# bowman-lab/enspara

Measured on AMD Instinct MI355X. Metric: frame x center RMSD pairs/sec in k-centers assign, higher is better.
Workload: dtype f32

## Files before the change

enspara_amd/_lib.py:

```python
import collections
import ctypes as C
import os

import numpy as np

HERE = os.path.dirname(os.path.abspath(__file__))
LIB_PATH = os.environ.get("ENSPARA_HIP_LIB",
                          os.path.join(HERE, "libenspara_hip.so"))

EK_TILE = 256
EK_OK, EK_EARG, EK_EHIP, EK_ESTATE, EK_ENOMEM = 0, -1, -2, -3, -4

SYMBOLS = [
    "ek_abi_version", "ek_last_error", "ek_device_count",
    "ek_ctx_create", "ek_ctx_destroy", "ek_ctx_sync", "ek_ctx_stream",
    "ek_load_frames", "ek_rmsd_to_center",
    "ek_state_reset", "ek_state_download", "ek_state_upload",
    "ek_record_bytes", "ek_local_candidate", "ek_own_record",
    "ek_kcenters_step", "ek_kcenters_run",
    "ek_history_download", "ek_history_reset",
    "ek_spec_candidates", "ek_round_candidates", "ek_quad_copy_ready",
    "ek_spec_begin", "ek_spec_round", "ek_spec_localmax",
    "ek_spec_apply", "ek_spec_round_end", "ek_spec_progress", "ek_spec_rounds",
    "ek_spec_chain_bytes", "ek_spec_chain_rows", "ek_spec_chain_max",
    "ek_spec_chain_apply", "ek_run_stats", "ek_ti_stats", "ek_view_stats",
    "ek_last_run_form",
    "ek_view_layout_check",
    "ek_ms_setup", "ek_ms_mailbox", "ek_ms_connect", "ek_ms_begin", "ek_ms_local",
    "ek_ms_global", "ek_ms_end", "ek_ms_run", "ek_ms_state", "ek_ms_diag",
    "ek_assign_nearest",
    "ek_pam_begin", "ek_pam_count_members", "ek_pam_select_member",
    "ek_pam_propose", "ek_pam_propose_member", "ek_pam_commit",
    "ek_pam_count_members_batch", "ek_pam_select_members_batch",
    "ek_pam_prefetch", "ek_pam_propose_ex", "ek_pam_prefetch_stats",
    "ek_pam_prefetch_window", "ek_pam_prefetch_passes", "ek_pam_sparse_stats", "ek_pam_ahead_stats", "ek_pam_window_run", "ek_pam_sweep", "ek_np_choice_draws",
    "ek_pam_window_max",
    "ek_pam_prefetch_centers_window",
    "ek_centered_frames", "ek_pam_begin_table", "ek_pam_prefetch_centers",
    "ek_pam_propose_center",
    "ek_msm_counts", "ek_msm_counts_ctx", "ek_msm_row_normalize",
    "ek_msm_mle_prinz", "ek_msm_bace_prune", "ek_msm_bace_run",
    "ek_msm_boot_open", "ek_msm_boot_fetch", "ek_msm_boot_build", "ek_msm_boot_last_timing",
    "ek_msm_boot_close",
    "ek_lu_solve", "ek_lu_set_timing", "ek_lu_last_timing",
    "ek_tpt_committors", "ek_tpt_mfpts_sinks", "ek_tpt_mfpts_all", "ek_tpt_fluxes",
    "ek_mi_open", "ek_mi_add", "ek_mi_load_counts", "ek_mi_counts", "ek_mi_information",
    "ek_mi_last_timing", "ek_mi_close",
    "ek_cards_open", "ek_cards_add", "ek_cards_stats", "ek_cards_disorder",
    "ek_cards_disorder_codes", "ek_cards_matrices", "ek_cards_counts",
    "ek_cards_last_timing", "ek_cards_close", "ek_cards_scan_chunk",
    "ek_sasa_open", "ek_sasa_run", "ek_sasa_last_timing", "ek_sasa_close",
    "ek_rmsf_open", "ek_rmsf_run", "ek_rmsf_fetch", "ek_rmsf_last_timing", "ek_rmsf_close",
    "ek_wmi_run", "ek_wmi_last_timing",
    "ek_ent_kl_rows", "ek_ent_js_rows", "ek_ent_shannon_rows", "ek_ent_kl_counts",
    "ek_ent_last_timing", "ek_ent_state_counts_open", "ek_ent_state_counts_add",
    "ek_ent_state_counts_read", "ek_ent_state_counts_last_timing",
    "ek_ent_state_counts_close",
    "ek_kmc_create", "ek_kmc_destroy", "ek_kmc_next", "ek_kmc_trajectories",
    "ek_kmc_ensemble", "ek_kmc_fret_probs", "ek_kmc_fret_bursts", "ek_kmc_last_timing",
    "ek_dye_pair_create", "ek_dye_pair_destroy", "ek_dye_pair_table", "ek_dye_pair_resolve",
    "ek_dye_pair_static", "ek_dye_pair_last_timing",
    "ek_dye_bursts_lifetimes", "ek_dye_bursts_k2", "ek_dye_photons_lifetimes",
    "ek_dye_photons_k2", "ek_dye_pick_events", "ek_dye_bursts_last_timing",
    "ek_pockets_open", "ek_pockets_run", "ek_pockets_counts", "ek_pockets_fetch",
    "ek_pockets_last_timing", "ek_pockets_close", "ek_pockets_touches", "ek_pockets_ranks",
    "ek_pockets_labels",
    "ek_dyes_open", "ek_dyes_run", "ek_dyes_counts", "ek_dyes_fetch", "ek_dyes_last_timing",
    "ek_dyes_close", "ek_dyes_touches", "ek_dyes_pair_hist",
    "ek_rotamer_states", "ek_dihedral_angles", "ek_dihedral_rotamers",
    "ek_krylov_create", "ek_krylov_destroy", "ek_krylov_set_vector",
    "ek_krylov_get_vector", "ek_krylov_step", "ek_krylov_rotate",
    "ek_krylov_combine", "ek_krylov_expand", "ek_krylov_set_filter",
    "ek_feat_create", "ek_feat_destroy", "ek_feat_load", "ek_feat_distance",
    "ek_feat_kcenters", "ek_feat_pam_sweep", "ek_feat_pam_release",
    "ek_feat_record_bytes", "ek_feat_create_sharded", "ek_feat_state_reset",
    "ek_feat_state_upload", "ek_feat_state_download", "ek_feat_local_candidate",
    "ek_feat_kcenters_step", "ek_feat_history_download", "ek_feat_history_reset",
    "ek_feat_pam_count_batch", "ek_feat_pam_select_batch", "ek_feat_pam_gather_rows",
    "ek_feat_pam_begin", "ek_feat_pam_propose", "ek_feat_pam_commit",
    "ek_feat_assign_nearest",
    "ek_set_frames_per_lane", "ek_set_option", "ek_get_option", "ek_last_run_timing",
    "ek_reserve_centers",
    "ek_debug_guards",
    "ek_timing_begin", "ek_timing_end", "ek_timing_form", "ek_hbm_copy_rate",
    "ek_qcp_probe", "ek_pam_pairs_probe",
    "ek_live_resources", "ek_fail_alloc_at",
]


EK_OPT_NONTEMPORAL = 1
EK_OPT_ASSIGN_KERNEL = 2
EK_OPT_CANDIDATES = 4
EK_OPT_CHAINED = 5
EK_OPT_PAM_PRUNE = 6
EK_OPT_STATE_EXACT = 7
EK_OPT_ADAPTIVE = 8
EK_OPT_PASS_FORM = 9
EK_OPT_FUSED_ROUNDS = 10
EK_OPT_TRIANGLE = 11
EK_OPT_PAM_ONE_WORKGROUP = 12
EK_OPT_PAM_MAX_PAIRS = 13
EK_OPT_PAM_BOTH_SUMS = 14
EK_OPT_FINE_PICK = 15
EK_OPT_PAM_BOUNDS = 16
EK_OPT_PICK_CAP = 17
EK_OPT_SMALL_SHARDS = 18
EK_OPT_PAM_AHEAD = 19
EK_OPT_PAM_ZERO_COPY = 20
EK_OPT_PAM_PAIRS_MFMA = 21
EK_OPT_PASS_SWEEP = 22
EK_OPT_MS_TWO_PHASE = 23
EK_OPT_ACTIVE_VIEW = 24
EK_OPT_VIEW_RHO = 25
EK_OPT_VIEW_RATIO = 26
OPTIONS = {k[7:].lower(): v for k, v in list(globals().items())
           if k.startswith("EK_OPT_")}


class HipLibraryMissing(RuntimeError):
    pass


class HipError(RuntimeError):
    pass


_lib = None


def load():
    global _lib
    if _lib is not None:
        return _lib
    if not os.path.exists(LIB_PATH):
        raise HipLibraryMissing(
            "%s not found: the HIP extension is not built "
            "(run `python -m enspara_amd.build`); there is no CPU fallback."
            % LIB_PATH)
    if os.environ.get("ENSPARA_NO_TORCH") != "1":
        try:
            import torch
        except Exception:
            pass
    try:
        L = C.CDLL(LIB_PATH, mode=C.RTLD_GLOBAL)
    except OSError as e:
        raise HipLibraryMissing("cannot load %s: %s" % (LIB_PATH, e))
    vp, i32, i64, f32 = C.c_void_p, C.c_int32, C.c_int64, C.c_float
    f32p, i32p, i64p = (C.POINTER(C.c_float), C.POINTER(C.c_int32),
                        C.POINTER(C.c_int64))
    L.ek_abi_version.restype = C.c_int
    L.ek_last_error.restype = C.c_char_p
    L.ek_device_count.restype = C.c_int
    L.ek_ctx_create.argtypes = [C.c_int, i64, i32, i64, vp, C.POINTER(vp)]
    L.ek_ctx_destroy.argtypes = [vp]
    L.ek_ctx_sync.argtypes = [vp]
    L.ek_ctx_stream.restype = vp
    L.ek_ctx_stream.argtypes = [vp]
    L.ek_load_frames.argtypes = [vp, vp, i64, i64, C.c_int]
    L.ek_rmsd_to_center.argtypes = [vp, i64, f32p, f32p]
    L.ek_state_reset.argtypes = [vp]
    L.ek_state_download.argtypes = [vp, f32p, i32p]
    L.ek_state_upload.argtypes = [vp, f32p, i32p]
    L.ek_record_bytes.restype = C.c_size_t
    L.ek_record_bytes.argtypes = [i32]
    L.ek_local_candidate.argtypes = [vp, vp]
    L.ek_own_record.restype = vp
    L.ek_own_record.argtypes = [vp]
    L.ek_kcenters_step.argtypes = [vp, vp, i32, i32, C.c_double, vp]
    L.ek_kcenters_run.argtypes = [vp, i32, i32, C.c_double, i32p, i64p, f32p, f32p]
    L.ek_history_download.argtypes = [vp, i32, i32, i64p, f32p, i32p]
    L.ek_history_reset.argtypes = [vp]
    L.ek_spec_candidates.argtypes = [vp]
    L.ek_round_candidates.argtypes = [vp]
    L.ek_quad_copy_ready.argtypes = [vp]
    L.ek_spec_begin.argtypes = [vp, i32, i32, vp]
    L.ek_spec_round.argtypes = [vp, vp, i32, C.c_double]
    L.ek_spec_localmax.argtypes = [vp, vp]
    L.ek_spec_apply.argtypes = [vp, vp, i32, C.c_double]
    L.ek_spec_chain_bytes.argtypes = [i32p, i32p]
    L.ek_spec_chain_rows.argtypes = [vp, vp]
    L.ek_spec_chain_max.argtypes = [vp, vp, i32, vp]
    L.ek_spec_chain_apply.argtypes = [vp, vp, i32, C.c_double]
    L.ek_spec_round_end.argtypes = [vp, vp]
    L.ek_spec_progress.argtypes = [vp, i32p, i32p]
    L.ek_spec_rounds.argtypes = [vp, i32p]
    L.ek_run_stats.argtypes = [vp, i64p, i64p]
    L.ek_ms_setup.argtypes = [vp, i32, i32, C.POINTER(C.c_size_t)]
    L.ek_ms_mailbox.argtypes = [vp, C.POINTER(vp), C.POINTER(vp), vp, vp]
    L.ek_ms_connect.argtypes = [vp, i32, vp, vp, vp, vp]
    L.ek_ms_begin.argtypes = [vp, i32, i32]
    L.ek_ms_local.argtypes = [vp, C.c_double, vp]
    L.ek_ms_global.argtypes = [vp, C.c_double, vp]
    L.ek_ms_end.argtypes = [vp]
    L.ek_ms_state.argtypes = [vp, i32p, i32p, i32p]
    L.ek_ms_run.argtypes = [vp, i32, i32, C.c_double, i32p, i64p, f32p, f32p]
    L.ek_ti_stats.argtypes = [vp, i64p, i64p]
    L.ek_view_stats.argtypes = [vp, i64p]
    L.ek_last_run_form.argtypes = [vp, i64p]
    L.ek_view_layout_check.argtypes = [vp, f32, i64p]
    L.ek_assign_nearest.argtypes = [vp, f32p, i32]
    f64p = C.POINTER(C.c_double)
    L.ek_ms_diag.argtypes = [vp, i64p, f64p]
    L.ek_pam_begin.argtypes = [vp, i64p, i32]
    L.ek_pam_count_members.argtypes = [vp, i32, i64p]
    L.ek_pam_select_member.argtypes = [vp, i32, i64, i64p]
    L.ek_pam_propose.argtypes = [vp, i32, i64, f64p, f64p, i64p]
    L.ek_pam_propose_member.argtypes = [vp, i32, i64, i64p, f64p, f64p, i64p]
    L.ek_pam_commit.argtypes = [vp, C.c_int]
    L.ek_pam_count_members_batch.argtypes = [vp, i32, i32, i64p]
    L.ek_pam_select_members_batch.argtypes = [vp, i32, i32, i64p, i64p]
    L.ek_pam_prefetch.argtypes = [vp, i64p, i32]
    L.ek_pam_propose_ex.argtypes = [vp, i32, i64, i64, i32, i32, f64p, f64p,
                                    i64p, C.POINTER(C.c_uint32)]
    L.ek_pam_prefetch_stats.argtypes = [vp, i64p, i64p]
    L.ek_pam_window_run.argtypes = [vp, i32, i32, i64p, i64p, i32, i32, i32p, i32p,
                                    f64p, f64p, i64p]
    L.ek_pam_window_max.argtypes = []
    L.ek_pam_window_max.restype = i32
    L.ek_pam_prefetch_window.argtypes = [vp, i64p, i32, i32, i32]
    L.ek_pam_prefetch_passes.argtypes = [vp, i64p, i64p]
    L.ek_pam_sparse_stats.argtypes = [vp, i64p, i64p]
    L.ek_pam_ahead_stats.argtypes = [vp, i64p]
    L.ek_np_choice_draws.argtypes = [C.POINTER(C.c_uint32), i64, i64p, i64p, i64, i64p]
    L.ek_np_choice_draws.restype = i64
    L.ek_pam_sweep.argtypes = [vp, i32, i32, C.POINTER(C.c_uint32), i64, i64p, i64p, i32p, i64p,
                               i32p, f64p, f64p, i64p, i32p]
    L.ek_pam_prefetch_centers_window.argtypes = [vp, vp, vp, i32, i32, i32]
    L.ek_centered_frames.argtypes = [vp, i64p, i32p, i32, vp, vp]
    L.ek_pam_begin_table.argtypes = [vp, vp, vp, i32]
    L.ek_pam_prefetch_centers.argtypes = [vp, vp, vp, i32]
    L.ek_pam_propose_center.argtypes = [vp, i32, i32, vp, vp, i64, i32, i32, vp]
    L.ek_msm_counts.argtypes = [C.c_int, i32p, i64p, i64, i32, i32, i32, i64,
                                i32p, i32p, i64p, i64p]
    L.ek_msm_counts_ctx.argtypes = [vp, i64p, i64, i32, i32, i32, i64, i32p, i32p,
                                    i64p, i64p]
    L.ek_msm_row_normalize.argtypes = [C.c_int, i64p, f64p, i64, f64p, f64p]
    L.ek_msm_mle_prinz.argtypes = [C.c_int, i32, i64, i32, i64p, i32p, i32p, f64p,
                                   f64p, f64p, f64p, f64p, f64p, f64p, C.c_double,
                                   i64, i64p, f64p]
    L.ek_msm_bace_prune.argtypes = [C.c_int, i32, f64p, f64p, f32p]
    L.ek_msm_bace_run.argtypes = [C.c_int, i32, f64p, f64p, i32p, i32, i32, i32, vp,
                                  i32, f32p]
    L.ek_msm_boot_open.argtypes = [C.c_int, i32p, i64p, i64, i32, i32, i32, i64, i64p, i32p,
                                   i32, i32p, i32, C.POINTER(vp)]
    L.ek_msm_boot_fetch.argtypes = [vp, i32, i32, i64p]
    L.ek_msm_boot_build.argtypes = [vp, i64, i64p, i64p, i64p, f64p, f64p]
    L.ek_msm_boot_last_timing.argtypes = [vp, f64p]
    L.ek_msm_boot_close.argtypes = [vp]
    L.ek_lu_solve.argtypes = [C.c_int, i32, f64p, i32, f64p, f64p, i32p, i32p]
    L.ek_lu_set_timing.argtypes = [C.c_int]
    L.ek_lu_last_timing.argtypes = [f64p, f64p]
    L.ek_tpt_committors.argtypes = [C.c_int, i32, f64p, i32p, i32, i32p, i32, f64p, i32p]
    L.ek_tpt_mfpts_sinks.argtypes = [C.c_int, i32, f64p, i32p, i32, C.c_double, f64p, i32p]
    L.ek_tpt_mfpts_all.argtypes = [C.c_int, i32, f64p, f64p, C.c_double, f64p, i32p]
    L.ek_tpt_fluxes.argtypes = [C.c_int, i32, f64p, i32p, i32, i32p, i32, f64p, i32, f64p,
                                f64p, i32p]
    u8p, u32p = C.POINTER(C.c_uint8), C.POINTER(C.c_uint32)
    L.ek_mi_open.argtypes = [C.c_int, i32, i32, i32, i32, C.POINTER(vp)]
    L.ek_mi_add.argtypes = [vp, u8p, u8p, i64]
    L.ek_mi_load_counts.argtypes = [vp, u32p, C.c_uint64]
    L.ek_mi_counts.argtypes = [vp, u32p]
    L.ek_mi_information.argtypes = [vp, f64p]
    L.ek_mi_last_timing.argtypes = [vp, f64p]
    L.ek_mi_close.argtypes = [vp]
    L.ek_cards_open.argtypes = [C.c_int, i32, i32, C.POINTER(vp)]
    L.ek_cards_add.argtypes = [vp, u8p, i64]
    L.ek_cards_stats.argtypes = [vp, i64p]
    L.ek_cards_disorder.argtypes = [vp, i64p, i64p]
    L.ek_cards_disorder_codes.argtypes = [vp, i32, u8p]
    L.ek_cards_matrices.argtypes = [vp, f64p]
    L.ek_cards_counts.argtypes = [vp, i32, u32p]
    L.ek_cards_last_timing.argtypes = [vp, f64p]
    L.ek_cards_close.argtypes = [vp]
    L.ek_cards_scan_chunk.argtypes = []
    L.ek_cards_scan_chunk.restype = C.c_int
    L.ek_sasa_open.argtypes = [C.c_int, i32, f32p, i32, f32p, i32, i32p, i32p, C.POINTER(vp)]
    L.ek_sasa_run.argtypes = [vp, f32p, i64, i64, i32p, f32p, f32p]
    L.ek_sasa_last_timing.argtypes = [vp, f64p]
    L.ek_sasa_close.argtypes = [vp]
    L.ek_rmsf_open.argtypes = [C.c_int, i32, i32, i32p, f32p, i32, i32p, i32p, C.POINTER(vp)]
    L.ek_rmsf_run.argtypes = [vp, f32p, i64, f64p, i64, i64, f32p, f64p, f32p,
                              C.POINTER(C.c_uint32)]
    L.ek_rmsf_fetch.argtypes = [vp, f64p, f64p]
    L.ek_rmsf_last_timing.argtypes = [vp, f64p]
    L.ek_rmsf_close.argtypes = [vp]
    L.ek_wmi_run.argtypes = [C.c_int, u8p, f64p, i64, i32, i32, f64p, f64p]
    L.ek_wmi_last_timing.argtypes = [f64p]
    L.ek_ent_kl_rows.argtypes = [C.c_int, i64, i64, f64p, f64p, f64p, u32p]
    L.ek_ent_js_rows.argtypes = [C.c_int, i64, i64, f64p, f64p, f64p, f64p, u32p]
    L.ek_ent_shannon_rows.argtypes = [C.c_int, i64, i64, f64p, i32, f64p]
    L.ek_ent_kl_counts.argtypes = [C.c_int, i32, f64p, i64, i32p, i32p, i64p, C.c_double,
                                   f64p, u32p]
    L.ek_ent_last_timing.argtypes = [f64p]
    L.ek_ent_state_counts_open.argtypes = [C.c_int, i32, i32, C.POINTER(vp)]
    L.ek_ent_state_counts_add.argtypes = [vp, u8p, i64]
    L.ek_ent_state_counts_read.argtypes = [vp, C.POINTER(C.c_uint64)]
    L.ek_ent_state_counts_last_timing.argtypes = [vp, f64p]
    L.ek_ent_state_counts_close.argtypes = [vp]
    u64 = C.c_uint64
    L.ek_kmc_create.argtypes = [C.c_int, i32, i64p, i32p, f64p, C.POINTER(vp)]
    L.ek_kmc_destroy.argtypes = [vp]
    L.ek_kmc_next.argtypes = [vp, i64, i32p, f64p, i32p, i64p]
    L.ek_kmc_trajectories.argtypes = [vp, u64, i64, i64, i32p, i64, i32, i64, i32p, i64p]
    L.ek_kmc_ensemble.argtypes = [C.c_int, i32, f64p, i64p, i32p, f64p, f64p, i64, f64p,
                                  f64p, f64p]
    L.ek_kmc_fret_probs.argtypes = [C.c_int, u64, i64, i64, i32p, i32, i64p, f64p, f64p,
                                    C.c_double, C.c_double, f64p]
    L.ek_kmc_fret_bursts.argtypes = [vp, u64, i64, i64, i64p, i64p, f64p, i64p, f64p, f64p,
                                     C.c_double, C.c_double, i64, u8p, i32p, i64p]
    L.ek_kmc_last_timing.argtypes = [f64p]
    i8p = C.POINTER(C.c_int8)
    L.ek_dye_pair_create.argtypes = [C.c_int, i32, i64p, i64p, i32p, f64p, f64p, f64p, i64p,
                                     i64p, i32p, f64p, f64p, f64p, f64p, C.POINTER(vp)]
    L.ek_dye_pair_destroy.argtypes = [vp]
    L.ek_dye_pair_table.argtypes = [vp, i32, f64p, f64p, f64p, f64p]
    L.ek_dye_pair_resolve.argtypes = [vp, u64, i64, i64, i64, i64, i32p, i8p, i32p, i32p, i64,
                                      i64p, i64p]
    L.ek_dye_pair_static.argtypes = [vp, u64, i64, i64, f64p, i8p, i32p, i32p]
    L.ek_dye_pair_last_timing.argtypes = [f64p]
    L.ek_dye_bursts_lifetimes.argtypes = [vp, u64, i64, i64, i64p, i64p, f64p, i64p, f64p, u8p,
                                          i64, u8p, f64p, i32p, i32p, i64p, i64p]
    L.ek_dye_bursts_k2.argtypes = [vp, u64, i64, i64, i64p, i64p, f64p, i64p, f64p, i64p, f64p,
                                   C.c_double, i64, u8p, f64p, f64p, i32p, i32p, i32p, i32p,
                                   i64p, i64p]
    L.ek_dye_photons_lifetimes.argtypes = [C.c_int, u64, i64, i64, i32p, i32, i64p, f64p, u8p,
                                           u8p, f64p, i64p]
    L.ek_dye_photons_k2.argtypes = [C.c_int, u64, i64, i64, i32p, i32, i64p, f64p, i64p, f64p,
                                    C.c_double, u8p, f64p, f64p, i32p, i32p, i64p]
    L.ek_dye_pick_events.argtypes = [C.c_int, i64, i32p, f64p, i32, i64p, i64p, i64p]
    L.ek_dye_bursts_last_timing.argtypes = [f64p]
    L.ek_pockets_open.argtypes = [C.c_int, i32, f64p, C.c_double, i32, C.POINTER(vp)]
    L.ek_pockets_run.argtypes = [vp, f32p, i64, f32p, i32p, i64]
    L.ek_pockets_counts.argtypes = [vp, i64, i64p]
    L.ek_pockets_fetch.argtypes = [vp, i32p, i32p]
    L.ek_pockets_last_timing.argtypes = [vp, f64p]
    L.ek_pockets_close.argtypes = [vp]
    L.ek_pockets_touches.argtypes = [C.c_int, f32p, i32, f64p, C.c_double, f32p, i32p, u8p]
    L.ek_pockets_ranks.argtypes = [C.c_int, u8p, i32p, u8p]
    L.ek_pockets_labels.argtypes = [C.c_int, u8p, i32p, i32p]
    L.ek_dyes_open.argtypes = [C.c_int, i32, f64p, i32, f32p, i32, f32p, C.c_double,
                               C.POINTER(vp)]
    L.ek_dyes_run.argtypes = [vp, f32p, i64, f32p, i64]
    L.ek_dyes_counts.argtypes = [vp, i64, i32p, i32p]
    L.ek_dyes_fetch.argtypes = [vp, i64p]
    L.ek_dyes_last_timing.argtypes = [vp, f64p]
    L.ek_dyes_close.argtypes = [vp]
    L.ek_dyes_touches.argtypes = [C.c_int, f32p, i32, f64p, f32p, i32, u8p]
    L.ek_dyes_pair_hist.argtypes = [C.c_int, f32p, i32, f32p, i32, C.c_double, i32p, i64p]
    L.ek_rotamer_states.argtypes = [C.c_int, f32p, i64, i32, u8p, i32, i32p, f64p, f32p,
                                    C.c_double, u8p, f64p]
    L.ek_dihedral_angles.argtypes = [C.c_int, f32p, i64, i32, i32p, i32, f32p, f64p]
# ... 113 lines not shown
```

enspara_amd/csrc/ek_api.hip:

```cpp
#include "ek_ctx.h"
#include "ek_view.h"
#include <cmath>
#include <mutex>
#include "ek_qcp.h"

static thread_local char g_err[512] = "";

int ek_set_error(int code, const char *fmt, ...)
{
    va_list ap;
    va_start(ap, fmt);
    vsnprintf(g_err, sizeof(g_err), fmt, ap);
    va_end(ap);
    return code;
}
void ek_ctx_msm_view(ek_ctx *c, int *device, int64_t *n, const int32_t **assign,
                     hipStream_t *stream, void ***scratch_slot)
{
    *device = c->device;
    *n = c->loaded ? c->n : -1;
    *assign = c->assign;
    *stream = c->stream;
    *scratch_slot = &c->msm_scratch;
}
// ... 125 lines not shown
    for (size_t k = 0; k < g_uc_live.size(); ++k)
        if (g_uc_live[k].ptr == ptr && g_uc_live[k].device == device) {
            g_uc_free.push_back(g_uc_live[k]);
            g_uc_live.erase(g_uc_live.begin() + k);
            return;
        }
}

bool ek_poison()
{
    static const bool on = getenv("EK_POISON") != nullptr;
    return on;
}
hipError_t ek_malloc_named(ek_ctx *c, void **ptr, size_t bytes, const char *name)
{
    if (!ek_poison())
        return ek_dev_malloc(ptr, bytes);
    hipError_t e = ek_dev_malloc(ptr, bytes + EK_GUARD_BYTES);
    static const int fill = getenv("EK_POISON_BYTE") ? (int)strtol(getenv("EK_POISON_BYTE"), nullptr, 0)
                                                     : 0x5a;
    if (e == hipSuccess)
        e = hipMemset(*ptr, fill, bytes);
    if (e == hipSuccess)
        e = hipMemset((unsigned char *)*ptr + bytes, 0xA5, EK_GUARD_BYTES);
    if (e == hipSuccess)
        e = hipDeviceSynchronize();
    if (e == hipSuccess)
        c->guards.push_back({name, (unsigned char *)*ptr + bytes});
    return e;
}
extern "C" int ek_debug_guards(ek_ctx *c)
{
    if (!c)
        return ek_fail(EK_EARG, "NULL context");
    EK_HIP(hipSetDevice(c->device));
    EK_HIP(hipDeviceSynchronize());
    int bad = 0;
    std::vector<unsigned char> h(EK_GUARD_BYTES);
    for (const ek_ctx::Guard &g : c->guards) {
        if (hipMemcpy(h.data(), g.at, EK_GUARD_BYTES, hipMemcpyDeviceToHost) != hipSuccess) {
            (void)hipGetLastError();
            continue;
        }
        for (size_t k = 0; k < h.size(); ++k)
            if (h[k] != 0xA5) {
                fprintf(stderr, "enspara_hip: buffer %s overrun: byte + %zu behind its end "
                                "is 0x%02x\n", g.name, k, h[k]);
                ++bad;
                break;
            }
    }
    return bad;
}

int ek_spec_alloc(ek_ctx *c)
{
    if (!c->top)
        EK_HIP(ek_malloc_named(c, (void **)&c->top, ek_top_scratch_bytes(c->A), "top"));
    if (!c->planD)
        EK_HIP(ek_malloc_named(c, (void **)&c->planD, 64 * 64 * sizeof(float), "planD"));
    if (!c->pm) {
        const size_t nb = ((size_t)std::max<int64_t>(c->n, 1) + EK_BLOCK - 1) /
                          EK_BLOCK;
        if (!c->fm)
            EK_HIP(ek_malloc_named(c, (void **)&c->fm, 4 * nb * sizeof(EkBlockMax), "fm"));
        EK_HIP(ek_malloc_named(c, (void **)&c->pm,
                               (size_t)(EK_MAX_CANDS - 1) * nb * sizeof(EkBlockMax), "pm"));
    }
    if (!c->vecs) {
        const size_t bytes = (size_t)(EK_MAX_CANDS - 1) * std::max<int64_t>(c->n_pad, 1) *
                             sizeof(float);
        EK_HIP(ek_malloc_named(c, (void **)&c->vecs, bytes, "vecs"));
    }
    return EK_OK;
}

extern "C" int ek_abi_version(void) { return EK_ABI_VERSION; }
extern "C" const char *ek_last_error(void) { return g_err; }

extern "C" int ek_device_count(void)
{
    int n = 0;
    hipError_t e = hipGetDeviceCount(&n);
    if (e != hipSuccess)
        return ek_fail(EK_EHIP, "hipGetDeviceCount: %s", hipGetErrorString(e));
    return n;
}

extern "C" size_t ek_record_bytes(int32_t n_atoms) { return ek_rec_bytes(n_atoms); }

int ek_free_all(ek_ctx *c)
{
    if (!c)
        return EK_OK;
    (void)hipSetDevice(c->device);
    if (c->stream)
        (void)hipStreamSynchronize(c->stream);
    (void)ek_dev_free(c->tiles);
    (void)ek_dev_free(c->qtiles);
    (void)ek_dev_free(c->aos);
    (void)ek_dev_free(c->G);
    (void)ek_dev_free(c->dist);
    (void)ek_dev_free(c->assign);
    (void)ek_dev_free(c->scratch);
    (void)ek_dev_free(c->rec);
    (void)ek_dev_free(c->rec_tmp);
    (void)ek_dev_free(c->blockmax);
    (void)ek_dev_free(c->hist);
    (void)ek_dev_free(c->ctl);
    for (int b = 0; b < 2; ++b) {
        (void)ek_dev_free(c->stage[b]);
        (void)ek_pinned_free(c->pin[b]);
        if (c->up_ev[b])
            (void)ek_event_destroy(c->up_ev[b]);
    }
    delete c->pool;
    (void)ek_dev_free(c->cen_aos);
    (void)ek_dev_free(c->cen_G);
    (void)ek_dev_free(c->cen_tiles);
    (void)ek_dev_free(c->cen_blocks);
    (void)ek_dev_free(c->bat_blockcnt);
    (void)ek_dev_free(c->bat_scan);
    (void)ek_dev_free(c->bat_sel);
    (void)ek_dev_free(c->pam_vecs);
    (void)ek_dev_free(c->pam_recs);
    (void)ek_dev_free(c->pam_plan);
    (void)ek_dev_free(c->moved);
    (void)ek_dev_free(c->tmp_idx);
    (void)ek_dev_free(c->pam_out_dev);
    (void)ek_dev_free(c->med_list);
    (void)ek_dev_free(c->dtab);
    if (c->act_n_host)
        (void)ek_pinned_free(c->act_n_host);
    if (c->pam_out_host)
        (void)ek_pinned_free(c->pam_out_host);
    (void)ek_dev_free(c->pam_win_dev);
    (void)ek_dev_free(c->sp_buf);
    (void)ek_dev_free(c->act_list);
    if (c->pam_win_host)
        (void)ek_pinned_free(c->pam_win_host);
    ek_msm_scratch_free(c->msm_scratch);
    for (void *m : c->ms_ipc)
        (void)hipIpcCloseMemHandle(m);
    (void)ek_dev_free(c->ms);
    ek_uncached_free(c->device, c->ms_mbox);
    ek_uncached_free(c->device, c->ms_flags);
    (void)ek_dev_free(c->recsT);
    (void)ek_dev_free(c->ctile);
    (void)ek_dev_free(c->ctrace);
    (void)ek_dev_free(c->ti_D);
    (void)ek_dev_free(c->ti_tab);
    (void)ek_dev_free(c->ti_tabG);
    (void)ek_dev_free(c->ti_skip);
    (void)ek_dev_free(c->ti_stats);
    (void)ek_dev_free(c->pend);
    (void)ek_dev_free(c->ord);
    (void)ek_dev_free(c->tick);
    (void)ek_dev_free(c->rows);
    (void)ek_dev_free(c->vmask);
    (void)ek_dev_free(c->plan);
    (void)ek_dev_free(c->vecs);
    (void)ek_dev_free(c->hdr);
    (void)ek_dev_free(c->pm);
    (void)ek_dev_free(c->ti_rtab);
    (void)ek_dev_free(c->ti_tmask);
    (void)ek_dev_free(c->pam_dprop);
    (void)ek_pinned_free(c->sel_host);
    (void)ek_pinned_free(c->cnt_host);
    (void)ek_pinned_free(c->js_host);
    (void)ek_dev_free(c->sp_marks);
    if (c->win_ev)
        (void)ek_event_destroy(c->win_ev);
    (void)ek_dev_free(c->fm);
    ek_view_free(c);
    (void)ek_dev_free(c->top);
    (void)ek_dev_free(c->planD);
    (void)ek_dev_free(c->ndist);
    (void)ek_dev_free(c->nassign);
    (void)ek_dev_free(c->amb);
    (void)ek_dev_free(c->amb_best);
    (void)ek_dev_free(c->amb_count);
    (void)ek_dev_free(c->blockcnt);
    (void)ek_dev_free(c->scan);
    (void)ek_dev_free(c->sel);
    (void)ek_dev_free(c->sq_part);
    (void)ek_dev_free(c->pw_shapes);
    (void)ek_dev_free(c->sq_out);
    (void)ek_dev_free(c->med_aos);
    (void)ek_dev_free(c->med_G);
    (void)ek_dev_free(c->med_idx);
    (void)ek_dev_free(c->ambt);
    (void)ek_dev_free(c->ambG);
    for (hipEvent_t e : c->samp_ev)
        (void)ek_event_destroy(e);
    if (c->ev0)
        (void)ek_event_destroy(c->ev0);
    if (c->ev1)
        (void)ek_event_destroy(c->ev1);
    if (c->evb0)
        (void)ek_event_destroy(c->evb0);
    if (c->evb1)
        (void)ek_event_destroy(c->evb1);
    if (c->own_stream && c->stream)
        (void)ek_stream_destroy(c->stream);
    delete c;
    return EK_OK;
}

extern "C" int ek_ctx_create(int device, int64_t n_frames, int32_t n_atoms,
                             int64_t global_offset, void *stream, ek_ctx **out)
{
    if (!out)
        return ek_fail(EK_EARG, "ek_ctx_create: out is NULL");
    *out = nullptr;
    if (n_frames < 0 || n_frames > 0x7fffff00LL)
        return ek_fail(EK_EARG, "ek_ctx_create: n_frames=%lld out of range",
                       (long long)n_frames);
    if (n_atoms < 1 || n_atoms > EK_MAX_ATOMS)
        return ek_fail(EK_EARG, "ek_ctx_create: n_atoms=%d out of range [1,%d]",
                       n_atoms, EK_MAX_ATOMS);
    EK_HIP(hipSetDevice(device));
    ek_ctx *c = new (std::nothrow) ek_ctx();
    if (!c)
        return ek_fail(EK_ENOMEM, "ek_ctx_create: out of host memory");
    c->device = device;
    c->n = n_frames;
    c->A = n_atoms;
    c->goff = global_offset;
    c->n_tiles = (n_frames + EK_TILE - 1) / EK_TILE;
    if (stream) {
        c->stream = (hipStream_t)stream;
    } else {
        hipError_t e = ek_stream_create_flags(&c->stream, hipStreamNonBlocking);
        if (e != hipSuccess) {
            delete c;
            return ek_fail(EK_EHIP, "ek_ctx_create: creating the stream: %s", hipGetErrorString(e));
        }
        c->own_stream = true;
    }
    const size_t tile_floats = (size_t)3 * n_atoms * EK_TILE;
    const size_t nn = (size_t)std::max<int64_t>(n_frames, 1);
    const size_t nt = (size_t)std::max<int64_t>(c->n_tiles, 1);
    const size_t recb = ek_rec_bytes(n_atoms);
    c->blockmax_cap = (int)((n_frames + EK_BLOCK - 1) / EK_BLOCK) + 1;
    c->hist_cap = 1024;
    hipError_t e = hipSuccess;
#define EK_ALLOC(ptr, bytes)                                                   \
    if (e == hipSuccess)                                                       \
        e = ek_malloc_named(c, (void **)&(ptr), (bytes), #ptr);
    EK_ALLOC(c->tiles, nt * tile_floats * sizeof(float));
    EK_ALLOC(c->aos, nn * (size_t)3 * n_atoms * sizeof(float));
    EK_ALLOC(c->G, nn * sizeof(double));
    EK_ALLOC(c->dist, nn * sizeof(float));
    EK_ALLOC(c->assign, nn * sizeof(int32_t));
    EK_ALLOC(c->scratch, nn * sizeof(float));
    EK_ALLOC(c->rec, recb);
    EK_ALLOC(c->rec_tmp, recb);
    EK_ALLOC(c->blockmax, (size_t)c->blockmax_cap * sizeof(EkBlockMax));
    EK_ALLOC(c->hist, (size_t)c->hist_cap * sizeof(EkHist));
    EK_ALLOC(c->ctl, sizeof(EkCtl));
    EK_ALLOC(c->recsT, recb * EK_MAX_CANDS);
    EK_ALLOC(c->plan, sizeof(EkPlan));
    EK_ALLOC(c->hdr, sizeof(EkMaxHdr));
    EK_ALLOC(c->pend, sizeof(EkPend));
    EK_ALLOC(c->ord, sizeof(EkChainOrd));
#ifdef EK_P16_STATS
    EK_ALLOC(c->tick, (256 + 64 * 16 + 2048) * sizeof(unsigned int));
    (void)hipMemset(c->tick, 0, (256 + 64 * 16 + 2048) * sizeof(unsigned int));
#else
    EK_ALLOC(c->tick, 256 * sizeof(unsigned int));
#endif
    EK_ALLOC(c->rows, EK_MAX_CANDS * sizeof(EkChainRow));
    EK_ALLOC(c->vmask, (nt * EK_TILE / EK_WAVE) * sizeof(uint32_t));
    EK_ALLOC(c->ctile, ek_ctile_bytes(n_atoms));
    EK_ALLOC(c->ctrace, EK_MAX_CANDS * sizeof(double));
#undef EK_ALLOC
    c->n_pad = (int64_t)nt * EK_TILE;
    if (e == hipSuccess)
        e = ek_event_create(&c->ev0);
    if (e == hipSuccess)
        e = ek_event_create(&c->ev1);
    if (e == hipSuccess && c->n_tiles > 0)
        e = hipMemsetAsync(c->tiles + (size_t)(c->n_tiles - 1) * tile_floats, 0,
                           tile_floats * sizeof(float), c->stream);
    if (e == hipSuccess)
        e = hipMemsetAsync(c->hist, 0, (size_t)c->hist_cap * sizeof(EkHist),
                           c->stream);
    if (e == hipSuccess)
        e = hipMemsetAsync(c->ctl, 0, sizeof(EkCtl), c->stream);
    if (e == hipSuccess)
        e = hipMemsetAsync(c->rec, 0, recb, c->stream);
    if (e == hipSuccess)
        e = hipMemsetAsync(c->pend, 0, sizeof(EkPend), c->stream);
    if (e == hipSuccess)
        e = hipMemsetAsync(c->plan, 0, sizeof(EkPlan), c->stream);
    if (e == hipSuccess)
        e = hipMemsetAsync(c->ord, 0, sizeof(EkChainOrd), c->stream);
    if (e == hipSuccess)
        e = hipMemsetAsync(c->tick, 0, 256 * sizeof(unsigned int), c->stream);
    if (e == hipSuccess)
        e = hipMemsetAsync(c->rows, 0, EK_MAX_CANDS * sizeof(EkChainRow),
                           c->stream);
    if (e != hipSuccess) {
        ek_free_all(c);
        return ek_fail(e == hipErrorOutOfMemory ? EK_ENOMEM : EK_EHIP,
                       "ek_ctx_create: %s", hipGetErrorString(e));
    }
    *out = c;
    return EK_OK;
}

extern "C" int ek_ctx_destroy(ek_ctx *ctx) { return ek_free_all(ctx); }

extern "C" int ek_ctx_sync(ek_ctx *c)
{
    if (!c)
        return ek_fail(EK_EARG, "NULL context");
    EK_HIP(hipSetDevice(c->device));
    EK_HIP(hipStreamSynchronize(c->stream));
    return EK_OK;
}

extern "C" void *ek_ctx_stream(ek_ctx *c) { return c ? (void *)c->stream : nullptr; }
extern "C" void *ek_own_record(ek_ctx *c) { return c ? (void *)c->rec : nullptr; }

extern "C" int ek_set_frames_per_lane(ek_ctx *c, int fpl)
{
    if (!c)
        return ek_fail(EK_EARG, "NULL context");
    if (fpl != 0 && fpl != 1 && fpl != 2 && fpl != 4)
        return ek_fail(EK_EARG, "frames per lane must be 0, 1, 2 or 4");
    c->fpl = fpl;
    return EK_OK;
}

extern "C" int ek_set_option(ek_ctx *c, int32_t key, int32_t value)
{
    if (!c)
        return ek_fail(EK_EARG, "NULL context");
    switch (key) {
    case EK_OPT_NONTEMPORAL:
        c->nt = value < 0 ? -1 : (value ? 1 : 0);
        return EK_OK;
    case EK_OPT_CANDIDATES:
        if (value != -1 && value != 1 && value != 4 && value != 8 && value != 16 &&
            value != 32)
            return ek_fail(EK_EARG, "ek_set_option: candidates per round must "
                                    "be -1 (auto), 1, 4, 8, 16 or 32");
        c->cands = value;
        return EK_OK;
    case EK_OPT_CHAINED:
        if (value != 0 && value != 1)
            return ek_fail(EK_EARG, "ek_set_option: chained rounds 0 or 1");
        c->chain = value;
        return EK_OK;
    case EK_OPT_PAM_PRUNE:
        if (value != 0 && value != 1)
            return ek_fail(EK_EARG, "ek_set_option: PAM medoid pruning 0 or 1");
        c->prune = value;
        return EK_OK;
    case EK_OPT_STATE_EXACT:
        if (value != 0 && value != 1)
            return ek_fail(EK_EARG, "ek_set_option: state-is-exact flag 0 or 1");
        c->state_exact = value != 0;
        return EK_OK;
    case EK_OPT_TRIANGLE:
        if (value != 0 && value != 1)
            return ek_fail(EK_EARG, "ek_set_option: triangle inequality 0 or 1");
        c->tri = value;
        return EK_OK;
    case EK_OPT_FUSED_ROUNDS:
        if (value != 0 && value != 1)
            return ek_fail(EK_EARG, "ek_set_option: fused rounds 0 or 1");
        c->fused = value;
        return EK_OK;
    case 9:
        if (value != 1)
            return ek_fail(EK_EARG, "ek_set_option: pass kernel form must be 1");
        return EK_OK;
    case EK_OPT_ADAPTIVE:
        if (value != 0 && value != 1)
            return ek_fail(EK_EARG, "ek_set_option: adaptive candidates 0 or 1");
        c->adapt = value;
        return EK_OK;
    case EK_OPT_PAM_ONE_WORKGROUP:
        if (value != 0 && value != 1)
            return ek_fail(EK_EARG, "ek_set_option: one-workgroup PAM windows 0 or 1");
        c->pam_sparse = value;
        return EK_OK;
    case EK_OPT_PAM_BOTH_SUMS:
        if (value != 0 && value != 1)
            return ek_fail(EK_EARG, "ek_set_option: both cost sums for every proposal 0 or 1");
        c->sp_exact = value;
        return EK_OK;
    case EK_OPT_PAM_MAX_PAIRS:
        if (value < 0)
            return ek_fail(EK_EARG, "ek_set_option: pairs one workgroup searches >= 0");
        c->sp_max_pairs = value;
        return EK_OK;
    case EK_OPT_PAM_PAIRS_MFMA:
        if (value != 0 && value != 1)
            return ek_fail(EK_EARG, "ek_set_option: PAM pairs kernels on the matrix cores 0 or 1");
        ek_pam_pairs_form = value;
        return EK_OK;
    case EK_OPT_PAM_ZERO_COPY:
        if (value != 0 && value != 1)
            return ek_fail(EK_EARG, "ek_set_option: PAM results into mapped host memory 0 or 1");
        c->pam_zero_copy = value;
        return EK_OK;
    case EK_OPT_PAM_AHEAD:
        if (value != 0 && value != 1)
            return ek_fail(EK_EARG, "ek_set_option: PAM slots evaluated ahead 0 or 1");
        c->pam_spec = value;
        return EK_OK;
    case EK_OPT_SMALL_SHARDS:
        if (value != 0 && value != 1)
            return ek_fail(EK_EARG, "ek_set_option: small shards 0 or 1");
        c->ms_small = value;
        return EK_OK;
    case EK_OPT_PICK_CAP:
        if (value < 0 || value > 16)
            return ek_fail(EK_EARG, "ek_set_option: far frames per label on the pick's list "
                                    "0 (by the yield) or 1 .. 16");
        c->pick_cap = value;
        return EK_OK;
    case EK_OPT_PAM_BOUNDS:
        if (value != 0 && value != 1)
            return ek_fail(EK_EARG, "ek_set_option: PAM tables as bounds 0 or 1");
        c->pam_bounds = value;
        return EK_OK;
    case EK_OPT_FINE_PICK:
        if (value != 0 && value != 1)
            return ek_fail(EK_EARG, "ek_set_option: maxima per 64 frames for the pick 0 or 1");
        c->fine_pick = value;
        return EK_OK;
    case EK_OPT_MS_TWO_PHASE:
        if (value != 0 && value != 1)
            return ek_fail(EK_EARG, "ek_set_option: headers first in the mailbox rounds 0 or 1");
        c->ms_two_phase = value;
        return EK_OK;
    case EK_OPT_PASS_SWEEP:
        if (value < 0 || value > 2)
// ... 247 lines not shown
        return ek_fail(EK_EARG, "NULL context");
    if (!c->loaded)
        return ek_fail(EK_ESTATE, "ek_state_reset: no frames loaded");
    EK_HIP(hipSetDevice(c->device));
    ek_launch_fill_state(c->dist, c->assign, c->n, __builtin_inff(), -1,
                         c->stream);
    EK_CHECK_LAUNCH();
    c->state_exact = true;
    ek_pam_forget(c);
    int rc = ek_history_reset(c);
    if (rc)
        return rc;
    return ek_local_candidate(c, nullptr);
}

extern "C" int ek_state_download(ek_ctx *c, float *dist_host,
                                 int32_t *assign_host)
{
    if (!c)
        return ek_fail(EK_EARG, "NULL context");
    EK_HIP(hipSetDevice(c->device));
    if (dist_host && c->n)
        EK_HIP(hipMemcpyAsync(dist_host, c->dist, (size_t)c->n * sizeof(float),
                              hipMemcpyDeviceToHost, c->stream));
    if (assign_host && c->n)
        EK_HIP(hipMemcpyAsync(assign_host, c->assign,
                              (size_t)c->n * sizeof(int32_t),
                              hipMemcpyDeviceToHost, c->stream));
    EK_HIP(hipStreamSynchronize(c->stream));
    return EK_OK;
}

extern "C" int ek_state_upload(ek_ctx *c, const float *dist_host,
                               const int32_t *assign_host)
{
    if (!c || !dist_host || !assign_host)
        return ek_fail(EK_EARG, "ek_state_upload: NULL argument");
    EK_HIP(hipSetDevice(c->device));
    if (c->n) {
        EK_HIP(hipMemcpyAsync(c->dist, dist_host, (size_t)c->n * sizeof(float),
                              hipMemcpyHostToDevice, c->stream));
        EK_HIP(hipMemcpyAsync(c->assign, assign_host,
                              (size_t)c->n * sizeof(int32_t),
                              hipMemcpyHostToDevice, c->stream));
    }
    EK_HIP(hipStreamSynchronize(c->stream));
    c->state_exact = false;
    ek_pam_forget(c);
    return ek_local_candidate(c, nullptr);
}

extern "C" int ek_local_candidate(ek_ctx *c, void *rec_dev)
{
    if (!c)
        return ek_fail(EK_EARG, "NULL context");
    if (!c->loaded)
        return ek_fail(EK_ESTATE, "ek_local_candidate: no frames loaded");
    EK_HIP(hipSetDevice(c->device));
    unsigned char *rec = rec_dev ? (unsigned char *)rec_dev : c->rec;
    ek_launch_pick(nullptr, 0, c->dist, c->tiles, c->G, c->n, c->A, c->goff,
                   rec, c->ctl, c->stream);
    EK_CHECK_LAUNCH();
    return EK_OK;
}

int ek_ensure_hist(ek_ctx *c, int32_t label)
{
    if (label < c->hist_cap)
        return EK_OK;
    int32_t cap = c->hist_cap;
    while (cap <= label)
        cap *= 2;
    EkHist *h = nullptr;
    hipError_t e = ek_dev_malloc((void **)&h, (size_t)cap * sizeof(EkHist));
    if (e == hipSuccess)
        e = hipMemsetAsync(h, 0, (size_t)cap * sizeof(EkHist), c->stream);
    if (e == hipSuccess)
        e = hipMemcpyAsync(h, c->hist, (size_t)c->hist_cap * sizeof(EkHist),
                           hipMemcpyDeviceToDevice, c->stream);
    if (e == hipSuccess)
        e = hipStreamSynchronize(c->stream);
    if (e != hipSuccess) {
        (void)hipStreamSynchronize(c->stream);
        (void)ek_dev_free(h);
        EK_HIP(e);
    }
    (void)ek_dev_free(c->hist);
    c->hist = h;
    c->hist_cap = cap;
    return EK_OK;
}

extern "C" int ek_kcenters_step(ek_ctx *c, const void *recs_dev, int32_t n_recs,
                                int32_t label, double dist_cutoff,
                                void *own_rec_out)
{
    if (!c)
        return ek_fail(EK_EARG, "NULL context");
    if (!c->loaded)
        return ek_fail(EK_ESTATE, "ek_kcenters_step: no frames loaded");
    if (label < 0)
        return ek_fail(EK_EARG, "ek_kcenters_step: negative label");
    EK_HIP(hipSetDevice(c->device));
    int rc = ek_ensure_hist(c, label);
    if (rc)
        return rc;
    const unsigned char *recs =
        recs_dev ? (const unsigned char *)recs_dev : c->rec;
    if (!recs_dev)
        n_recs = 1;
    if (n_recs < 1)
        return ek_fail(EK_EARG, "ek_kcenters_step: n_recs < 1");
    unsigned char *own = own_rec_out ? (unsigned char *)own_rec_out : c->rec;
    const int fpl = ek_pick_fpl(c);
    bool tri = false;
    if (c->tri && recs_dev && c->state_exact && c->A >= 3) {
        if (label == 0)
            c->ti_tab_n = 0;
        if (c->ti_tab_n == label) {
            if (label + 1 > c->ti_tab_cap) {
                const int32_t cap = std::max(2 * c->ti_tab_cap, std::max(label + 1, 256));
                float *t2 = nullptr, *d2 = nullptr;
                double *g2 = nullptr;
                EK_HIP(ek_wait(c));
                hipError_t e = ek_dev_malloc((void **)&t2, (size_t)cap * 3 * c->A * sizeof(float));
                if (e == hipSuccess)
                    e = ek_dev_malloc((void **)&g2, (size_t)cap * sizeof(double));
                if (e == hipSuccess)
                    e = ek_dev_malloc((void **)&d2, (size_t)cap * sizeof(float));
                if (e == hipSuccess && c->ti_tab_n > 0)
                    e = hipMemcpy(t2, c->ti_tab, (size_t)c->ti_tab_n * 3 * c->A * sizeof(float),
                                  hipMemcpyDeviceToDevice);
                if (e == hipSuccess && c->ti_tab_n > 0)
                    e = hipMemcpy(g2, c->ti_tabG, (size_t)c->ti_tab_n * sizeof(double),
                                  hipMemcpyDeviceToDevice);
                if (e != hipSuccess) {
                    (void)ek_dev_free(t2);
                    (void)ek_dev_free(g2);
                    (void)ek_dev_free(d2);
                    EK_HIP(e);
                }
                (void)ek_dev_free(c->ti_tab);
                (void)ek_dev_free(c->ti_tabG);
                (void)ek_dev_free(c->ti_D);
                c->ti_tab = t2;
                c->ti_tabG = g2;
                c->ti_D = d2;
                c->ti_tab_cap = cap;
                c->ti_cap = cap;
            }
            if (!c->ti_skip)
                EK_HIP(ek_dev_malloc((void **)&c->ti_skip,
                                     (size_t)std::max<int64_t>(c->n_tiles, 1)));
            if (!c->ti_stats) {
                EK_HIP(ek_dev_malloc((void **)&c->ti_stats, 2 * sizeof(unsigned long long)));
                EK_HIP(hipMemsetAsync(c->ti_stats, 0, 2 * sizeof(unsigned long long),
                                      c->stream));
            }
            if (label == 0)
                EK_HIP(hipMemsetAsync(c->ti_stats, 0, 2 * sizeof(unsigned long long),
                                      c->stream));
            ek_launch_ti_tab(c->ti_tab, c->ti_tabG, c->A, label, recs, n_recs, c->ti_D,
                             c->dist, c->assign, c->n, c->ctl, c->ti_skip, c->ti_stats,
                             c->stream);
            EK_CHECK_LAUNCH();
            c->ti_tab_n = label + 1;
            tri = label >= 1 && c->n > 0;
        }
    }
    if (c->n > 0) {
        const bool sample =
            c->samp_every > 0 && (c->samp_count++ % c->samp_every) == 0 &&
            2 * (size_t)c->samp_used + 1 < c->samp_ev.size();
        if (sample)
        c->samp_form[c->samp_used] = 1;
    if (sample)
            EK_HIP(hipEventRecord(c->samp_ev[2 * c->samp_used], c->stream));
        ek_launch_step(fpl, 0, ek_pick_nt(c), c->tiles, c->G, c->dist, c->assign, c->scratch,
                       recs, n_recs, c->n, c->A, label, dist_cutoff,
                       c->blockmax, c->hist, c->ctl, c->stream,
                       tri ? c->ti_skip : nullptr);
        EK_CHECK_LAUNCH();
        if (sample) {
            EK_HIP(hipEventRecord(c->samp_ev[2 * c->samp_used + 1], c->stream));
            c->samp_used++;
        }
    }
    ek_launch_pick(c->n > 0 ? c->blockmax : nullptr,
                   ek_step_blocks(fpl, c->n), c->dist, c->tiles, c->G, c->n,
                   c->A, c->goff, own, c->ctl, c->stream);
    EK_CHECK_LAUNCH();
    return EK_OK;
}

extern "C" int ek_history_download(ek_ctx *c, int32_t first, int32_t count,
                                   int64_t *center_index_out,
                                   float *center_dist_out, int32_t *n_done)
{
    if (!c)
        return ek_fail(EK_EARG, "NULL context");
    if (first < 0 || count < 0)
        return ek_fail(EK_EARG, "ek_history_download: bad range");
    EK_HIP(hipSetDevice(c->device));
    EkCtl ctl;
    EK_HIP(hipMemcpyAsync(&ctl, c->ctl, sizeof(ctl), hipMemcpyDeviceToHost,
                          c->stream));
    std::vector<EkHist> h;
    const int32_t avail = std::max(0, std::min(count, c->hist_cap - first));
    if (avail > 0) {
        h.resize(avail);
        EK_HIP(hipMemcpyAsync(h.data(), c->hist + first,
                              (size_t)avail * sizeof(EkHist),
                              hipMemcpyDeviceToHost, c->stream));
    }
    EK_HIP(ek_wait(c));
    for (int32_t i = 0; i < count; ++i) {
        const bool ok = i < avail && h[i].set;
        if (center_index_out)
            center_index_out[i] = ok ? h[i].gidx : -1;
        if (center_dist_out)
            center_dist_out[i] = ok ? h[i].dist : 0.f;
    }
    if (n_done)
        *n_done = ctl.n_done;
    return EK_OK;
}

extern "C" int ek_timing_begin(ek_ctx *c, int32_t sample_every,
                               int32_t max_samples)
{
    if (!c || sample_every < 1 || max_samples < 1)
        return ek_fail(EK_EARG, "ek_timing_begin: bad argument");
    EK_HIP(hipSetDevice(c->device));
    while (c->samp_ev.size() < 2 * (size_t)max_samples) {
        hipEvent_t e;
        EK_HIP(ek_event_create(&e));
        c->samp_ev.push_back(e);
    }
    c->samp_form.assign((size_t)max_samples, 0);
    c->samp_every = sample_every;
    c->samp_used = 0;
    c->samp_count = 0;
    return EK_OK;
}

extern "C" int ek_timing_end(ek_ctx *c, float *avg_ms, int32_t *n_samples)
{
    if (!c)
        return ek_fail(EK_EARG, "NULL context");
    EK_HIP(hipSetDevice(c->device));
    EK_HIP(ek_wait(c));
    int cnt[EK_MAX_CANDS + 1] = {0};
    for (int i = 0; i < c->samp_used; ++i)
        cnt[std::min(std::max(c->samp_form[i], 0), EK_MAX_CANDS)]++;
    int dom = 0;
    for (int f = 1; f <= EK_MAX_CANDS; ++f)
        if (cnt[f] > cnt[dom])
            dom = f;
    c->samp_dom = dom;
    std::vector<float> t((size_t)c->samp_used);
    float mx = 0.f;
    for (int i = 0; i < c->samp_used; ++i) {
        EK_HIP(hipEventElapsedTime(&t[i], c->samp_ev[2 * i],
                                   c->samp_ev[2 * i + 1]));
        if (c->samp_form[i] == dom)
            mx = std::max(mx, t[i]);
    }
    double sum = 0.0;
    int used = 0;
    for (int i = 0; i < c->samp_used; ++i)
        if (c->samp_form[i] == dom && t[i] > 0.25f * mx) {
            sum += t[i];
            ++used;
        }
    if (avg_ms)
        *avg_ms = used ? (float)(sum / used) : 0.f;
    if (n_samples)
        *n_samples = used;
    c->samp_every = 0;
    return EK_OK;
}

extern "C" int ek_timing_form(ek_ctx *c, int32_t *candidates)
{
    if (!c || !candidates)
        return ek_fail(EK_EARG, "ek_timing_form: NULL argument");
    *candidates = c->samp_dom;
    return EK_OK;
}

extern "C" int ek_assign_nearest(ek_ctx *c, const float *centers_xyz,
                                 int32_t n_centers)
{
    if (!c || (!centers_xyz && n_centers > 0))
        return ek_fail(EK_EARG, "ek_assign_nearest: NULL argument");
    if (!c->loaded)
        return ek_fail(EK_ESTATE, "ek_assign_nearest: no frames loaded");
    if (n_centers < 0)
        return ek_fail(EK_EARG, "ek_assign_nearest: negative n_centers");
    if ((size_t)3 * c->A * 8 * sizeof(float) > 150 * 1024)
        return ek_fail(EK_EARG, "ek_assign_nearest: %d atoms exceed the LDS "
                                "center tile (limit 1600)", c->A);
    EK_HIP(hipSetDevice(c->device));
    c->state_exact = false;
    ek_pam_forget(c);
    if (n_centers > 0) {
        int rc = ek_upload_centers(c, centers_xyz, n_centers);
        if (rc)
            return rc;
    }
    const bool mfma = c->assign_variant == 2 || c->assign_variant == 3 ||
// ... 211 lines not shown
```

enspara_amd/csrc/ek_api_run.hip:

```cpp
#include "ek_ctx.h"
#include "ek_run_policy.h"
#include "ek_view.h"
#include <cmath>

void ek_view_free(ek_ctx *c)
{
    (void)ek_dev_free(c->v_aos);
    (void)ek_dev_free(c->v_tiles);
    (void)ek_dev_free(c->v_qtiles);
    (void)ek_dev_free(c->v_G);
    (void)ek_dev_free(c->v_dist);
    (void)ek_dev_free(c->v_assign);
    (void)ek_dev_free(c->v_act);
    (void)ek_dev_free(c->v_blockcnt);
    (void)ek_dev_free(c->v_blockoff);
    (void)ek_dev_free(c->v_count);
    c->v_aos = c->v_tiles = c->v_qtiles = nullptr;
    c->v_G = nullptr;
    c->v_dist = nullptr;
    c->v_assign = nullptr;
    c->v_act = c->v_blockcnt = c->v_blockoff = c->v_count = nullptr;
    c->view_cap = 0;
}

// ... 3 lines not shown
    if (c->view_cap >= cap)
        return EK_OK;
    EK_HIP(ek_wait(c));
    ek_view_free(c);
    const size_t nt = (size_t)(cap / EK_TILE), A3 = (size_t)3 * c->A;
    const size_t nblk = ek_view_sel_blocks(std::max<int64_t>(c->n, 1));
    hipError_t e = hipSuccess;
#define EK_VALLOC(ptr, bytes)                                                  \
    if (e == hipSuccess)                                                       \
        e = ek_malloc_named(c, (void **)&(ptr), (bytes), #ptr);
    EK_VALLOC(c->v_aos, (size_t)cap * A3 * sizeof(float));
    EK_VALLOC(c->v_tiles, nt * A3 * EK_TILE * sizeof(float));
    EK_VALLOC(c->v_qtiles, ek_quad_tiles_bytes((int64_t)nt, c->A));
    EK_VALLOC(c->v_G, (size_t)cap * sizeof(double));
    EK_VALLOC(c->v_dist, (size_t)cap * sizeof(float));
    EK_VALLOC(c->v_assign, (size_t)cap * sizeof(int32_t));
    EK_VALLOC(c->v_act, (size_t)cap * sizeof(uint32_t));
    EK_VALLOC(c->v_blockcnt, nblk * sizeof(uint32_t));
    EK_VALLOC(c->v_blockoff, nblk * sizeof(uint32_t));
    EK_VALLOC(c->v_count, 2 * sizeof(uint32_t));
    if (e == hipSuccess)
        e = hipMemsetAsync(c->v_count, 0, 2 * sizeof(uint32_t), c->stream);
#undef EK_VALLOC
    if (e != hipSuccess) {
        (void)hipGetLastError();
        ek_view_free(c);
        if (e == hipErrorOutOfMemory) {
            c->view_nomem = true;
            return EK_ENOMEM;
        }
        EK_HIP(e);
    }
    c->view_cap = cap;
    return EK_OK;
}

struct EkViewRun {
    bool on = false;
    int64_t n = 0;
    int32_t label_lo = 0;
    double guard = 0.0;
    bool tiles_valid = false;
};

static hipError_t ek_view_poison(ek_ctx *c)
{
    const size_t cap = (size_t)c->view_cap, nt = cap / EK_TILE, A3 = (size_t)3 * c->A;
    hipError_t e = hipMemsetAsync(c->v_aos, 0xFF, cap * A3 * sizeof(float), c->stream);
    if (e == hipSuccess)
        e = hipMemsetAsync(c->v_tiles, 0xFF, nt * A3 * EK_TILE * sizeof(float), c->stream);
    if (e == hipSuccess)
        e = hipMemsetAsync(c->v_qtiles, 0xFF, ek_quad_tiles_bytes((int64_t)nt, c->A),
                           c->stream);
    if (e == hipSuccess)
        e = hipMemsetAsync(c->v_G, 0xFF, cap * sizeof(double), c->stream);
    if (e == hipSuccess)
        e = hipMemsetAsync(c->v_dist, 0xFF, cap * sizeof(float), c->stream);
    if (e == hipSuccess)
        e = hipMemsetAsync(c->v_assign, 0xFF, cap * sizeof(int32_t), c->stream);
    return e;
}

static bool ek_view_build(ek_ctx *c, int64_t n_v)
{
    ek_launch_view_build(c->v_act, n_v, c->A, c->qt_valid, c->aos, c->G, c->dist, c->assign,
                         c->v_aos, c->qt_valid ? c->v_qtiles : c->v_tiles, c->v_G, c->v_dist,
                         c->v_assign, c->stream);
    return !c->qt_valid;
}

static void ek_view_scatter_back(ek_ctx *c, EkViewRun &v)
{
    ek_launch_view_scatter(c->v_act, v.n, c->v_dist, c->v_assign, c->dist, c->assign,
                           c->hist, v.label_lo, c->hist_cap, c->ctl, c->goff, c->stream);
    v.on = false;
}

void ek_round_of(ek_ctx *c, int T, double cutoff, EkRound &R)
{
    R.dist = c->dist;
    R.assign = c->assign;
    R.vecs = c->vecs;
    R.n = c->n;
    R.n_pad = c->n_pad;
    R.goff = c->goff;
    R.A = c->A;
    R.T = T;
    R.tiles = c->tiles;
    R.qtiles = c->qtiles;
    R.aos = c->aos;
    R.G = c->G;
    R.recs = c->recsT;
    R.plan = c->plan;
    R.pend = c->pend;
    R.ord = c->ord;
    R.blockmax = c->blockmax;
    R.pm = c->pm;
    R.fm = c->fine_pick ? c->fm : nullptr;
    R.sweep = (c->pass_sweep == 2 ||
               (c->pass_sweep == 1 && ek_sweep_pays(c->n))) ? 1 : 0;
    R.top = c->top;
    R.ctile = c->ctile;
    R.ctrace = c->ctrace;
    R.hist = c->hist;
    R.ctl = c->ctl;
    R.tick = c->tick;
    R.rows = c->rows;
    R.vmask = c->vmask;
    R.cutoff = cutoff;
    R.pick_cap = c->pick_cap > 0 ? c->pick_cap : 4;
}

static void ek_note_run_form(ek_ctx *c, int fpl, int nt, bool fused, int Tmax, int sweep,
                             bool fine_buf)
{
    const int nb = (int)((c->n + EK_BLOCK - 1) / EK_BLOCK);
    const bool fine = fused && Tmax > 1 && fine_buf && ek_fine_fits(nb);
    c->last_form[0] = fpl;
    c->last_form[1] = nt ? 1 : 0;
    c->last_form[2] = sweep ? 1 : 0;
    c->last_form[3] = fine ? 1 : 0;
    c->last_form[4] = nb;
    c->last_form[5] = Tmax > 1 ? (fine ? 4 * (int64_t)nb : nb) : ek_step_blocks(fpl, c->n);
}

#define EK_RC(call)                                                            \
    do {                                                                       \
        const int rc_ = (call);                                                \
        if (rc_)                                                               \
            return rc_;                                                        \
    } while (0)

struct EkRun {
    ek_ctx *c;
    EkViewRun &view;
    int32_t first_label, goal;
    double dist_cutoff;
    bool tri;
    bool fused;
    int fpl, nt;
    int view_mode;
    bool forced;
    double rho, shrink;
    EkRound R;
    int nb = 0;
    EkFormLadder lad;
    EkPickCap cap;
    EkTriPause ti;
    EkViewPolicy vp;
    int held = -1;
    bool pending = false;
    bool masks_fresh = false;
    bool looked = false;
    uint32_t look_cnt[2] = {0, 0};
    EkCtl cr;
    double per_round;
    int32_t rounds_before = 0;
    EkRun(ek_ctx *c_, EkViewRun &view_, bool adaptive, bool tri_, int Tmax)
        : c(c_), view(view_), tri(tri_), lad(adaptive, tri_, Tmax), cap(c_->pick_cap),
          per_round(ek_per_round_guess(lad.form))
    {
        memset(&cr, 0, sizeof(cr));
    }
};

static int ek_run_reserve_tri(ek_ctx *c, int32_t goal)
{
    if (goal > c->ti_cap) {
        EK_HIP(ek_wait(c));
        (void)ek_dev_free(c->ti_D);
        c->ti_D = nullptr;
        c->ti_cap = 0;
        EK_HIP(ek_dev_malloc((void **)&c->ti_D, (size_t)(goal + 1) * sizeof(float)));
        c->ti_cap = goal + 1;
    }
    if (!c->ti_skip)
        EK_HIP(ek_dev_malloc((void **)&c->ti_skip,
                             (size_t)std::max<int64_t>(c->n_tiles, 1)));
    if (!c->ti_stats)
        EK_HIP(ek_dev_malloc((void **)&c->ti_stats, 2 * sizeof(unsigned long long)));
    EK_HIP(hipMemsetAsync(c->ti_stats, 0, 2 * sizeof(unsigned long long),
                          c->stream));
    if (goal > c->ti_rtab_cap) {
        EK_HIP(ek_wait(c));
        (void)ek_dev_free(c->ti_rtab);
        c->ti_rtab = nullptr;
        c->ti_rtab_cap = 0;
        EK_HIP(ek_dev_malloc((void **)&c->ti_rtab,
                         (size_t)(goal + 1) * EK_MAX_CANDS * sizeof(float)));
        c->ti_rtab_cap = goal + 1;
    }
    if (!c->ti_tmask)
        EK_HIP(ek_dev_malloc((void **)&c->ti_tmask,
                         (size_t)std::max<int64_t>(c->n_tiles, 1) * sizeof(uint32_t)));
    return EK_OK;
}

static void ek_run_use_store(EkRun &run, bool the_view)
{
    ek_ctx *c = run.c;
    EkRound &R = run.R;
    if (the_view) {
        R.dist = c->v_dist;
        R.assign = c->v_assign;
        R.tiles = c->v_tiles;
        R.qtiles = c->v_qtiles;
        R.aos = c->v_aos;
        R.G = c->v_G;
        R.n = run.view.n;
        R.n_pad = (run.view.n + EK_TILE - 1) / EK_TILE * EK_TILE;
    } else {
        R.dist = c->dist;
        R.assign = c->assign;
        R.tiles = c->tiles;
        R.qtiles = c->qtiles;
        R.aos = c->aos;
        R.G = c->G;
        R.n = c->n;
        R.n_pad = c->n_pad;
    }
    run.nb = (int)((R.n + EK_BLOCK - 1) / EK_BLOCK);
    R.sweep = (run.fused && (c->pass_sweep == 2 ||
                             (c->pass_sweep == 1 && ek_sweep_pays(R.n)))) ? 1 : 0;
    R.cutoff = the_view ? std::max(run.dist_cutoff, run.view.guard) : run.dist_cutoff;
}

static void ek_run_leave_view(EkRun &run)
{
    if (run.pending) {
        ek_launch_round_flush(run.R, run.c->stream);
        run.pending = false;
    }
    ek_view_scatter_back(run.c, run.view);
    ek_run_use_store(run, false);
}

static int ek_run_enter_view(EkRun &run, int32_t left)
{
    ek_ctx *c = run.c;
    EkViewRun &view = run.view;
    run.looked = false;
    const EkViewPlan p =
        run.vp.decide(run.cr.last_max, run.rho, run.shrink, run.look_cnt,
                      view.on ? view.n : 0, c->n, left, run.per_round, run.forced);
    if (!p.build)
        return EK_OK;
    if (view.on) {
        ek_run_leave_view(run);
    } else if (run.pending) {
        ek_launch_round_flush(run.R, c->stream);
        run.pending = false;
    }
    uint32_t nv = 0;
    ek_launch_view_select(c->dist, c->n, p.theta, c->v_blockcnt, c->v_blockoff, c->v_act,
                          c->view_cap, c->v_count, c->stream);
    EK_CHECK_LAUNCH();
    EK_HIP(hipMemcpyAsync(&nv, c->v_count, sizeof(nv), hipMemcpyDeviceToHost, c->stream));
    EK_HIP(ek_wait(c));
    if (nv > 0 && (int64_t)nv < c->n && (int64_t)nv <= c->view_cap) {
        view.n = nv;
        view.label_lo = run.cr.n_done;
        view.guard = p.guard;
        if (run.view_mode == 3)
            EK_HIP(ek_view_poison(c));
        view.tiles_valid = ek_view_build(c, view.n);
        EK_CHECK_LAUNCH();
        view.on = true;
        ek_run_use_store(run, true);
        EK_HIP(hipMemsetAsync(c->vmask, 0, (size_t)(run.R.n_pad / EK_WAVE) * sizeof(uint32_t),
                              c->stream));
        c->view_stats[0]++;
    }
    run.held = -1;
    return EK_OK;
}

static void ek_run_pick_records(EkRun &run, int form, bool with_masks)
{
    ek_ctx *c = run.c;
    const EkRound &R = run.R;
    if (form == 1) {
        ek_launch_pick(c->blockmax, run.nb, R.dist, R.tiles, R.G, R.n, c->A, c->goff,
                       c->recsT, c->ctl, c->stream);
    } else if (run.fused) {
        ek_launch_round_chain(R, 1, c->stream);
        ek_launch_round_next(R, 1, c->stream);
        if (with_masks) {
            ek_launch_round_ti(R, run.goal, c->stream);
            run.masks_fresh = R.tmask != nullptr;
        }
    } else {
        ek_launch_pickT(c->blockmax, run.nb, R.tiles, R.G, R.assign, c->A, form, c->goff,
                        c->recsT, c->ctl, c->top, c->stream);
    }
}

static int ek_run_bootstrap(EkRun &run, int form)
{
    ek_ctx *c = run.c;
    if (run.pending) {
        ek_launch_round_flush(run.R, c->stream);
        run.pending = false;
    } else if (run.held <= 1) {
        ek_launch_blockmax(run.R.dist, run.R.n, c->blockmax, c->stream);
    }
    ek_run_pick_records(run, form, true);
    EK_CHECK_LAUNCH();
    if (form != 1)
        run.per_round = ek_per_round_guess(form);
    run.held = form;
    return EK_OK;
}

static int ek_run_enqueue_steps(EkRun &run, int32_t batch)
{
    ek_ctx *c = run.c;
    const EkRound &R = run.R;
    for (int32_t r = 0; r < batch; ++r) {
        const int label = run.cr.n_done + r;
        const bool skip = run.tri && label >= 1;
        if (skip)
            ek_launch_ti(R.aos, R.G, c->A, c->hist, label, c->goff, c->recsT, c->ti_D, R.dist,
                         R.assign, R.n, c->ctl, c->ti_skip, c->ti_stats, c->stream);
        ek_launch_step(run.fpl, 0, run.nt, R.tiles, R.G, R.dist, R.assign, c->scratch,
                       c->recsT, 1, R.n, c->A, label, R.cutoff, c->blockmax, c->hist, c->ctl,
                       c->stream, skip ? c->ti_skip : nullptr);
        ek_launch_pick(c->blockmax, ek_step_blocks(run.fpl, R.n), R.dist, R.tiles, R.G, R.n,
                       c->A, c->goff, c->recsT, c->ctl, c->stream);
        EK_CHECK_LAUNCH();
    }
    return EK_OK;
}

static bool ek_run_sample(EkRun &run, int form)
{
    ek_ctx *c = run.c;
    const bool sample =
        !run.view.on && c->samp_every > 0 && (c->samp_count++ % c->samp_every) == 0 &&
        2 * (size_t)c->samp_used + 1 < c->samp_ev.size();
    if (sample)
        c->samp_form[c->samp_used] = form;
    return sample;
}

static int ek_run_enqueue_fused(EkRun &run, int form, int32_t batch)
{
    ek_ctx *c = run.c;
    const EkRound &R = run.R;
    for (int32_t r = 0; r < batch; ++r) {
        const bool sample = ek_run_sample(run, form);
        if (sample)
            EK_HIP(hipEventRecord(c->samp_ev[2 * c->samp_used], c->stream));
        ek_launch_round_pass(R, c->stream);
        if (sample) {
            EK_HIP(hipEventRecord(c->samp_ev[2 * c->samp_used + 1], c->stream));
            c->samp_used++;
        }
        ek_launch_round_chain(R, 0, c->stream);
        ek_launch_round_next(R, 0, c->stream);
        ek_launch_round_ti(R, run.goal, c->stream);
        EK_CHECK_LAUNCH();
        run.pending = true;
    }
    return EK_OK;
}

static int ek_run_enqueue_unfused(EkRun &run, int form, int32_t batch)
{
    ek_ctx *c = run.c;
    const EkRound &R = run.R;
    const int nb = run.nb;
    for (int32_t r = 0; r < batch; ++r) {
        const bool sample = ek_run_sample(run, form);
        ek_launch_plan(c->recsT, form, c->A, form, R.cutoff, c->planD, c->plan, c->hist,
                       c->ctl, c->stream);
        if (sample)
            EK_HIP(hipEventRecord(c->samp_ev[2 * c->samp_used], c->stream));
        ek_launch_pass(form, R.tiles, R.qtiles, R.G, R.dist, R.assign, c->vecs, R.n, R.n_pad,
                       c->A, c->recsT, c->plan, c->blockmax, c->ctile, c->ctrace, c->stream);
        if (sample) {
            EK_HIP(hipEventRecord(c->samp_ev[2 * c->samp_used + 1], c->stream));
            c->samp_used++;
        }
        if (c->chain) {
            ek_launch_chain_max(R.dist, c->vecs, R.n, R.n_pad, c->plan, c->pm, 1, c->goff,
                                c->stream);
            ek_launch_chain_decide_local(c->blockmax, c->pm, nb, ek_chain_max_blocks(R.n),
                                         c->goff, R.cutoff, c->plan, c->hist, c->ctl,
                                         c->stream);
            ek_launch_chain_apply(c->vecs, R.n, R.n_pad, R.dist, R.assign, c->plan,
                                  c->blockmax, c->stream);
        } else {
            for (int j = 1; j < form; ++j) {
                ek_launch_localmax_check(c->blockmax, nb, c->goff, R.cutoff, c->plan, c->hist,
                                         c->ctl, c->stream);
                ek_launch_apply(c->vecs, R.G, R.n, R.n_pad, c->A, R.dist, R.assign, c->plan,
                                c->blockmax, c->stream);
            }
        }
        ek_launch_pickT(c->blockmax, nb, R.tiles, R.G, R.assign, c->A, form, c->goff, c->recsT,
                        c->ctl, c->top, c->stream);
        EK_CHECK_LAUNCH();
    }
    return EK_OK;
}

static int ek_run_enqueue_batch(EkRun &run, int form, int32_t batch)
{
    const EkRound &R = run.R;
    if (R.tmask && !run.masks_fresh) {
        ek_launch_round_ti(R, run.goal, run.c->stream);
        run.masks_fresh = true;
    }
    if (!R.tmask)
        run.masks_fresh = false;
    if (form == 1)
        return ek_run_enqueue_steps(run, batch);
    return run.fused ? ek_run_enqueue_fused(run, form, batch)
                     : ek_run_enqueue_unfused(run, form, batch);
}

static int ek_run_carry_look(EkRun &run)
{
    ek_ctx *c = run.c;
    if (!run.view_mode || run.vp.pause.tick())
        return EK_OK;
    const int64_t want_cap =
        run.forced ? c->n : (int64_t)std::ceil(run.shrink * (double)c->n);
    if (ek_view_alloc(c, want_cap) != EK_OK) {
        (void)hipGetLastError();
        run.view_mode = 0;
        return EK_OK;
    }
    EK_HIP(hipMemsetAsync(c->v_count, 0, sizeof(run.look_cnt), c->stream));
    ek_launch_view_look(run.R.dist, run.R.n, c->ctl, run.rho, EK_VIEW_REL, EK_VIEW_ABS,
                        c->v_count, c->stream);
    if (run.view.on)
        ek_launch_view_look(c->dist, c->n, c->ctl, run.rho, EK_VIEW_REL, EK_VIEW_ABS,
                            c->v_count + 1, c->stream);
    EK_CHECK_LAUNCH();
    EK_HIP(hipMemcpyAsync(run.look_cnt, c->v_count, sizeof(run.look_cnt),
                          hipMemcpyDeviceToHost, c->stream));
    run.looked = true;
    return EK_OK;
}

static int ek_run_read_back(EkRun &run, int form, int32_t &got, int32_t &ran)
{
    ek_ctx *c = run.c;
    const bool one = form == 1, masks = run.R.tmask != nullptr;
    const int32_t before = run.cr.n_done;
    EK_HIP(hipMemcpyAsync(&run.cr, c->ctl, sizeof(run.cr), hipMemcpyDeviceToHost, c->stream));
    unsigned long long ti_now[2] = {0, 0};
    if (masks)
        EK_HIP(hipMemcpyAsync(ti_now, c->ti_stats, sizeof(ti_now), hipMemcpyDeviceToHost,
                              c->stream));
    EK_HIP(ek_wait(c));
    if (masks)
        run.ti.look(ti_now);
    else if (!one)
        run.ti.skipped();
    got = run.cr.n_done - before;
    ran = one ? got : run.cr.n_rounds - run.rounds_before;
    run.rounds_before = run.cr.n_rounds;
    c->st_rounds[ek_form_slot(form)] += ran;
    c->st_centers[ek_form_slot(form)] += got;
    c->view_stats[1] += (int64_t)ran * run.R.n;
    c->view_stats[2] += (int64_t)ran * (c->n - run.R.n);
    return EK_OK;
}

static int ek_run_leave_on_stop(EkRun &run)
{
    ek_ctx *c = run.c;
    if ((double)run.cr.last_max > run.dist_cutoff)
        c->view_stats[3]++;
    ek_run_leave_view(run);
    const int32_t zero = 0;
    EK_HIP(hipMemcpyAsync(&c->ctl->stopped, &zero, sizeof(zero), hipMemcpyHostToDevice,
                          c->stream));
    EK_HIP(ek_wait(c));
    run.cr.stopped = 0;
    run.held = -1;
    run.looked = false;
    return EK_OK;
}

static int ek_run_finish(EkRun &run, int32_t max_new, int32_t *n_added,
                         int64_t *center_index_out, float *center_dist_out,
                         float *final_maxdist)
{
    ek_ctx *c = run.c;
    const int form = run.lad.form;
    if (run.pending) {
        ek_launch_round_flush(run.R, c->stream);
        run.pending = false;
        EK_CHECK_LAUNCH();
    }
    if (run.view.on || (run.held < 0 && run.cr.n_done > run.first_label)) {
        if (run.view.on)
            ek_run_leave_view(run);
        ek_launch_blockmax(run.R.dist, run.R.n, c->blockmax, c->stream);
        run.R.T = form;
        ek_run_pick_records(run, form, false);
        EK_CHECK_LAUNCH();
        run.held = form;
        EK_HIP(hipMemcpyAsync(&run.cr, c->ctl, sizeof(run.cr), hipMemcpyDeviceToHost,
                              c->stream));
        EK_HIP(ek_wait(c));
    }
    if (run.tri) {
        unsigned long long st[2] = {0, 0};
        EK_HIP(hipMemcpyAsync(st, c->ti_stats, sizeof(st), hipMemcpyDeviceToHost, c->stream));
        EK_HIP(ek_wait(c));
        c->ti_tiles = (int64_t)st[0];
        c->ti_skipped = (int64_t)st[1];
    }
    EK_HIP(hipEventRecord(c->ev1, c->stream));
    EK_HIP(ek_wait(c));
    EK_HIP(hipEventElapsedTime(&c->last_ms, c->ev0, c->ev1));
    if (run.held == 1) {
        ek_launch_blockmax(c->dist, c->n, c->blockmax, c->stream);
        EK_CHECK_LAUNCH();
    }
    if (run.held >= 0)
        EK_HIP(hipMemcpyAsync(c->rec, c->recsT, ek_rec_bytes(c->A), hipMemcpyDeviceToDevice,
                              c->stream));
    EK_HIP(ek_wait(c));
    const int32_t added_t =
        std::min(max_new, std::max(0, run.cr.n_done - run.first_label));
    const int64_t passes = c->st_rounds[0] + c->st_rounds[1] + c->st_rounds[2] +
                           c->st_rounds[3] + 2 * c->st_rounds[4];
    c->last_launches = (int32_t)passes;
    c->last_passes = (int32_t)passes;
    if (n_added)
        *n_added = added_t;
    if (final_maxdist)
        *final_maxdist = run.cr.last_max;
    if (added_t > 0 && (center_index_out || center_dist_out))
        EK_RC(ek_history_download(c, run.first_label, added_t, center_index_out,
                                  center_dist_out, nullptr));
    return EK_OK;
}

static int ek_run_rounds_in(ek_ctx *c, int Tmax, int32_t first_label,
                            int32_t max_new, double dist_cutoff, int32_t *n_added,
                            int64_t *center_index_out, float *center_dist_out,
                            float *final_maxdist, EkViewRun &view)
{
    EK_RC(ek_spec_alloc(c));
    if (!c->evb0) {
        EK_HIP(ek_event_create(&c->evb0));
        EK_HIP(ek_event_create(&c->evb1));
    }
    const int32_t goal = first_label + max_new;
    EkCtl ctlw;
    memset(&ctlw, 0, sizeof(ctlw));
    ctlw.n_done = first_label;
    ctlw.limit = goal;
    EK_HIP(hipMemcpyAsync(c->ctl, &ctlw, sizeof(ctlw), hipMemcpyHostToDevice,
                          c->stream));
    EK_HIP(ek_wait(c));
    for (int m = 0; m < EK_N_FORMS; ++m)
        c->st_rounds[m] = c->st_centers[m] = 0;
    c->view_stats[0] = c->view_stats[1] = c->view_stats[2] = c->view_stats[3] = 0;
    const bool tri = c->tri && c->state_exact && first_label == 0 && c->A >= 3;
    if (tri)
        EK_RC(ek_run_reserve_tri(c, goal));
    c->ti_tiles = c->ti_skipped = 0;
    const bool fused = c->fused && c->chain == 1;
    if (Tmax == 32 && !fused)
        Tmax = EK_LEGACY_CANDS;
    if (Tmax >= 16) {
        const int eq = ek_ensure_qtiles(c);
        if (eq == EK_ENOMEM)
            Tmax = 8;
        else if (eq != EK_OK)
            return eq;
    }
    const bool adaptive = c->cands == -1 && c->adapt;
    const int view_mode =
        (c->state_exact && c->A >= 3 && fused && !c->tri && !c->view_nomem) ? c->active_view
                                                                             : 0;
    EkRun run(c, view, adaptive, tri, Tmax);
    run.first_label = first_label;
    run.goal = goal;
    run.dist_cutoff = dist_cutoff;
    run.fused = fused;
    run.fpl = ek_pick_fpl(c);
    run.nt = ek_pick_nt(c);
    run.view_mode = view_mode;
    run.forced = view_mode >= 2;
    run.rho = c->view_rho / 1000.0;
    run.shrink = c->view_ratio / 1000.0;
    run.cr.n_done = first_label;
    EkRound &R = run.R;
    ek_round_of(c, Tmax, dist_cutoff, R);
    R.ti_tab = tri ? c->ti_rtab : nullptr;
    R.ti_stats = tri ? c->ti_stats : nullptr;
    ek_run_use_store(run, false);
    ek_note_run_form(c, run.fpl, run.nt, fused, Tmax, R.sweep && Tmax == 16, R.fm != nullptr);
    EK_HIP(hipEventRecord(c->ev0, c->stream));
    while (run.cr.n_done < goal) {
        const int32_t left = goal - run.cr.n_done;
        const int form = run.lad.form;
        const bool one = form == 1;
        R.T = form;
        const bool masks = tri && fused && form >= 4 && !run.ti.paused();
        R.tmask = masks ? c->ti_tmask : nullptr;
        R.pick_cap = run.cap.cap;
        if (run.view_mode && run.looked && std::isfinite(run.cr.last_max))
            EK_RC(ek_run_enter_view(run, left));
        run.looked = false;
        if (view.on && !view.tiles_valid && form < 16) {
            ek_launch_view_tiles(c->v_qtiles, R.n_pad / EK_TILE, c->A, c->v_tiles, c->stream);
            EK_CHECK_LAUNCH();
            view.tiles_valid = true;
        }
        if (run.held != form)
            EK_RC(ek_run_bootstrap(run, form));
        const int32_t batch =
            ek_batch_single(form, left, run.lad.due(left), run.per_round, run.lad.probing,
                            run.forced, !run.view_mode ? 0 : (run.vp.pause.left > 0 ? 2 : 1));
        EK_HIP(hipEventRecord(c->evb0, c->stream));
        EK_RC(ek_run_enqueue_batch(run, form, batch));
        EK_HIP(hipEventRecord(c->evb1, c->stream));
        EK_RC(ek_run_carry_look(run));
        int32_t got = 0, ran = 0;
        EK_RC(ek_run_read_back(run, form, got, ran));
        if (view.on && run.cr.stopped) {
            EK_RC(ek_run_leave_on_stop(run));
            if (run.cr.n_done < goal)
                continue;
        }
        if (run.cr.stopped || run.cr.n_done >= goal)
            break;
        if (!one)
            run.per_round = std::max(1.0, (double)got / std::max(ran, 1));
        if (!one && fused && !run.lad.probing)
            run.cap.update(form, got, ran, left);
        if (!adaptive)
            continue;
        float bms = 0.f;
        EK_HIP(hipEventElapsedTime(&bms, c->evb0, c->evb1));
        run.lad.update(got, bms, run.per_round);
    }
    return ek_run_finish(run, max_new, n_added, center_index_out, center_dist_out,
                         final_maxdist);
}

static int ek_run_rounds(ek_ctx *c, int Tmax, int32_t first_label,
                         int32_t max_new, double dist_cutoff, int32_t *n_added,
                         int64_t *center_index_out, float *center_dist_out,
                         float *final_maxdist)
{
    EkViewRun view;
    const int rc = ek_run_rounds_in(c, Tmax, first_label, max_new, dist_cutoff, n_added,
                                    center_index_out, center_dist_out, final_maxdist, view);
    if (rc != EK_OK && view.on) {
        ek_view_scatter_back(c, view);
        (void)hipStreamSynchronize(c->stream);
        (void)hipGetLastError();
    }
    return rc;
}

extern "C" int ek_kcenters_run(ek_ctx *c, int32_t first_label, int32_t max_new,
                               double dist_cutoff, int32_t *n_added,
                               int64_t *center_index_out,
                               float *center_dist_out, float *final_maxdist)
{
    if (!c)
        return ek_fail(EK_EARG, "NULL context");
    if (!c->loaded)
        return ek_fail(EK_ESTATE, "ek_kcenters_run: no frames loaded");
    if (first_label < 0 || max_new < 0)
        return ek_fail(EK_EARG, "ek_kcenters_run: negative argument");
    EK_HIP(hipSetDevice(c->device));
    int rc = ek_ensure_hist(c, first_label + max_new);
    if (rc)
        return rc;
    EkCtl ctl0;
    memset(&ctl0, 0, sizeof(ctl0));
    ctl0.n_done = first_label;
    EK_HIP(hipMemcpyAsync(c->ctl, &ctl0, offsetof(EkCtl, last_max),
                          hipMemcpyHostToDevice, c->stream));
    EK_HIP(ek_wait(c));

    const int T = ek_pick_cands(c, true);
    if ((T > 1 || c->tri) && c->n > 0)
        return ek_run_rounds(c, T, first_label, max_new, dist_cutoff, n_added,
                             center_index_out, center_dist_out, final_maxdist);

    ek_note_run_form(c, ek_pick_fpl(c), ek_pick_nt(c), false, 1, 0, false);
    c->view_stats[0] = c->view_stats[1] = c->view_stats[2] = c->view_stats[3] = 0;
    const bool open_loop = !(dist_cutoff > 0.0);
    const int32_t batch = open_loop ? max_new : 16;
    int32_t issued = 0;
    EkCtl ctl;
    memset(&ctl, 0, sizeof(ctl));
    ctl.n_done = first_label;
    EK_HIP(hipEventRecord(c->ev0, c->stream));
    while (issued < max_new) {
        const int32_t todo = std::min(batch, max_new - issued);
        for (int32_t i = 0; i < todo; ++i) {
            rc = ek_kcenters_step(c, nullptr, 1, first_label + issued + i,
                                  dist_cutoff, nullptr);
            if (rc)
                return rc;
        }
        issued += todo;
        if (!open_loop) {
            EK_HIP(hipMemcpyAsync(&ctl, c->ctl, sizeof(ctl),
                                  hipMemcpyDeviceToHost, c->stream));
            EK_HIP(ek_wait(c));
            if (ctl.stopped)
                break;
        }
    }
    EK_HIP(hipEventRecord(c->ev1, c->stream));
    EK_HIP(hipMemcpyAsync(&ctl, c->ctl, sizeof(ctl), hipMemcpyDeviceToHost,
                          c->stream));
    EK_HIP(ek_wait(c));
    EK_HIP(hipEventElapsedTime(&c->last_ms, c->ev0, c->ev1));
    const int32_t added = std::max(0, ctl.n_done - first_label);
    c->last_launches = added;
    if (n_added)
        *n_added = added;
    if (final_maxdist)
        *final_maxdist = ctl.last_max;
    if (added > 0 && (center_index_out || center_dist_out)) {
        rc = ek_history_download(c, first_label, added, center_index_out,
                                 center_dist_out, nullptr);
        if (rc)
            return rc;
    }
    return EK_OK;
}

extern "C" int ek_view_layout_check(ek_ctx *c, float theta, int64_t *out)
{
    if (!c || !out)
        return ek_fail(EK_EARG, "ek_view_layout_check: NULL argument");
    if (!c->loaded || c->n <= 0)
        return ek_fail(EK_ESTATE, "ek_view_layout_check: no frames loaded");
    EK_HIP(hipSetDevice(c->device));
    out[0] = out[1] = out[2] = out[3] = 0;
    int rc = ek_view_alloc(c, c->n);
    if (rc)
        return rc;
    uint32_t nv = 0;
    ek_launch_view_select(c->dist, c->n, theta, c->v_blockcnt, c->v_blockoff, c->v_act,
                          c->view_cap, c->v_count, c->stream);
    EK_CHECK_LAUNCH();
    EK_HIP(hipMemcpyAsync(&nv, c->v_count, sizeof(nv), hipMemcpyDeviceToHost, c->stream));
    EK_HIP(ek_wait(c));
    out[0] = nv;
    if (nv == 0 || (int64_t)nv > c->view_cap)
        return EK_OK;
    const size_t nt = ((size_t)nv + EK_TILE - 1) / EK_TILE, A3 = (size_t)3 * c->A;
    const size_t tile_words = nt * A3 * EK_TILE;
    const size_t quad_bytes = ek_quad_tiles_bytes((int64_t)nt, c->A);
    float *r_aos = nullptr, *r_tiles = nullptr, *r_qtiles = nullptr, *r_dist = nullptr;
    double *r_G = nullptr;
    int32_t *r_assign = nullptr;
    unsigned long long *diff = nullptr, got[3] = {0, 0, 0};
    hipError_t e = ek_dev_malloc((void **)&r_aos, (size_t)nv * A3 * sizeof(float));
    if (e == hipSuccess)
        e = ek_dev_malloc((void **)&r_tiles, tile_words * sizeof(float));
    if (e == hipSuccess)
        e = ek_dev_malloc((void **)&r_qtiles, quad_bytes);
    if (e == hipSuccess)
        e = ek_dev_malloc((void **)&r_G, (size_t)nv * sizeof(double));
    if (e == hipSuccess)
        e = ek_dev_malloc((void **)&r_dist, (size_t)nv * sizeof(float));
    if (e == hipSuccess)
        e = ek_dev_malloc((void **)&r_assign, (size_t)nv * sizeof(int32_t));
    if (e == hipSuccess)
        e = ek_dev_malloc((void **)&diff, sizeof(got));
    if (e == hipSuccess)
        e = hipMemsetAsync(diff, 0, sizeof(got), c->stream);
    if (e == hipSuccess)
        e = ek_view_poison(c);
    if (e == hipSuccess) {
        ek_launch_view_gather(c->v_act, nv, c->A, c->aos, c->G, c->dist, c->assign, r_aos,
                              r_tiles, r_G, r_dist, r_assign, c->stream);
        ek_launch_quad_tiles(r_tiles, (int64_t)nt, c->A, r_qtiles, c->stream);
        if (!ek_view_build(c, nv))
            ek_launch_view_tiles(c->v_qtiles, (int64_t)nt, c->A, c->v_tiles, c->stream);
        if (c->qt_valid)
            ek_launch_view_diff(c->v_qtiles, r_qtiles, quad_bytes / 4, diff, c->stream);
        ek_launch_view_diff(c->v_tiles, r_tiles, tile_words, diff + 1, c->stream);
        ek_launch_view_diff(c->v_aos, r_aos, (size_t)nv * A3, diff + 2, c->stream);
        ek_launch_view_diff(c->v_G, r_G, (size_t)nv * 2, diff + 2, c->stream);
        ek_launch_view_diff(c->v_dist, r_dist, (size_t)nv, diff + 2, c->stream);
        ek_launch_view_diff(c->v_assign, r_assign, (size_t)nv, diff + 2, c->stream);
        e = hipGetLastError();
    }
    if (e == hipSuccess)
        e = hipMemcpyAsync(got, diff, sizeof(got), hipMemcpyDeviceToHost, c->stream);
    if (e == hipSuccess)
        e = ek_wait(c);
    else
        (void)hipStreamSynchronize(c->stream);
    (void)ek_dev_free(r_aos);
    (void)ek_dev_free(r_tiles);
    (void)ek_dev_free(r_qtiles);
    (void)ek_dev_free(r_G);
    (void)ek_dev_free(r_dist);
    (void)ek_dev_free(r_assign);
    (void)ek_dev_free(diff);
    EK_HIP(e);
    out[1] = (int64_t)got[0];
    out[2] = (int64_t)got[1];
    out[3] = (int64_t)got[2];
    return EK_OK;
}

extern "C" int ek_last_run_form(ek_ctx *c, int64_t *out)
{
    if (!c || !out)
        return ek_fail(EK_EARG, "ek_last_run_form: NULL argument");
    for (int k = 0; k < 6; ++k)
        out[k] = c->last_form[k];
    return EK_OK;
}

extern "C" int ek_view_stats(ek_ctx *c, int64_t *stats)
{
    if (!c || !stats)
        return ek_fail(EK_EARG, "ek_view_stats: NULL argument");
    for (int k = 0; k < 4; ++k)
        stats[k] = c->view_stats[k];
    return EK_OK;
}
```

enspara_amd/csrc/ek_common.h:

```cpp
#pragma once
#include <hip/hip_runtime.h>
#include <stdint.h>
#include <stddef.h>

#include "../../include/enspara_hip.h"
#include "ek_track.h"
#include "ek_pam_limits.h"

#define EK_BLOCK 256
#define EK_WAVE 64
#define EK_MAX_ATOMS 4096

struct EkRecHdr {
    float maxdist;
    int32_t valid;
    int64_t gidx;
    double trace;
    int64_t reserved;
};
static_assert(sizeof(EkRecHdr) == 32, "record header is 32 bytes");

static inline __host__ __device__ size_t ek_rec_bytes(int A)
{
    return (sizeof(EkRecHdr) + (size_t)12 * (size_t)A + 15) & ~(size_t)15;
}

struct EkBlockMax {
    float val;
    uint32_t idx;
};

struct EkHist {
    int64_t gidx;
    float dist;
    int32_t set;
};

struct EkCtl {
    int32_t n_done;
    int32_t stopped;
    float last_max;
    int32_t limit;
    int32_t n_rounds;
    int32_t pad[3];
};

struct EkMaxHdr {
    float maxdist;
    int32_t valid;
    int64_t gidx;
};
static_assert(sizeof(EkMaxHdr) == 16, "max header is 16 bytes");

typedef float ek_v2f __attribute__((ext_vector_type(2)));
#define EK_MAX_CANDS 32
#define EK_LEGACY_CANDS 16
#define EK_RED_THREADS 1024
__host__ __device__ inline bool ek_sweep_pays(int64_t n)
{
    return n <= (int64_t)2048 * EK_TILE;
}
__host__ __device__ inline bool ek_fine_fits(int nb)
{
    return 4 * nb <= 8 * EK_RED_THREADS;
}
struct EkPlan {
    int32_t go;
    int32_t teff;
    int32_t label;
    int32_t apply;
    int32_t apply_label;
    int32_t miss;
    uint32_t used;
    int32_t n_rec;
    int32_t src[EK_MAX_CANDS];
    int64_t gidx[EK_MAX_CANDS];
    float maxdist[EK_MAX_CANDS];
    double trace[EK_MAX_CANDS];
    int32_t chain_n;
    int32_t napply;
    int32_t chain_label0;
    int32_t pad2;
    int32_t chain[EK_MAX_CANDS];
    int32_t offer[EK_MAX_CANDS];
};

struct EkChainRow {
    float cur;
    int32_t valid;
    float d[EK_MAX_CANDS];
};
static_assert(sizeof(EkChainRow) == 8 + 4 * EK_MAX_CANDS, "EkChainRow layout");

struct EkPend {
    int32_t n;
    int32_t label0;
    int32_t slot[EK_MAX_CANDS];
};
struct EkChainOrd {
    int32_t n;
    int32_t cand[EK_MAX_CANDS];
};
struct EkFuse {
    const EkPend *pend = nullptr;
    EkChainOrd *ord = nullptr;
    unsigned int *tick = nullptr;
    int64_t goff = 0;
    EkHist *hist = nullptr;
    EkCtl *ctl = nullptr;
    EkChainRow *rows = nullptr;
    uint32_t *vmask = nullptr;
    const uint32_t *tmask = nullptr;
    EkBlockMax *sweep_pm = nullptr;
    EkBlockMax *sweep_fm = nullptr;
    int sweep_nb = 0;
};
struct EkRound {
    float *dist;
    int32_t *assign;
    float *vecs;
    int64_t n, n_pad, goff;
    int A, T;
    const float *tiles;
    const float *qtiles;
    const float *aos;
    const double *G;
    unsigned char *recs;
    EkPlan *plan;
    EkPend *pend;
    EkChainOrd *ord;
    EkBlockMax *blockmax;
    EkBlockMax *pm;
    EkBlockMax *fm;
    unsigned char *top;
    float *ctile;
    double *ctrace;
    EkHist *hist;
    EkCtl *ctl;
    EkChainRow *rows;
    uint32_t *vmask;
    unsigned int *tick;
    double cutoff;
    float *ti_tab = nullptr;
    uint32_t *tmask = nullptr;
    unsigned long long *ti_stats = nullptr;
    int pick_cap = 4;
    int sweep = 0;
};
void ek_launch_round_ti(const EkRound &r, int max_labels, hipStream_t s);
void ek_launch_round_pass(const EkRound &r, hipStream_t s, bool with_order = true);
void ek_launch_round_chain(const EkRound &r, int bootstrap, hipStream_t s);
void ek_launch_round_next(const EkRound &r, int bootstrap, hipStream_t s);
void ek_launch_round_flush(const EkRound &r, hipStream_t s);

#define EK_MS_MAX_WORLD 64
#ifndef EK_MS_SLOTS
#define EK_MS_SLOTS 128
#endif
struct EkMsMsg {
    int32_t n_recs;
    int32_t cn;
    int32_t state;
    int32_t pad;
};
static inline __host__ __device__ size_t ek_ms_msg_bytes(int A, int offer)
{
    return sizeof(EkMsMsg) + EK_MAX_CANDS * sizeof(EkMaxHdr) +
           (size_t)offer * ek_rec_bytes(A);
}
struct EkMsState {
    int32_t mode;
    int32_t pick_state;
    uint32_t seq;
    int32_t err;
    uint32_t err_seq;
    uint32_t n_reoffer;
    unsigned long long wait_ticks_max;
    unsigned long long wait_ticks_own;
};
struct EkMsXchg {
    int32_t world = 1, rank = 0, offer = 0;
    int32_t sys = 0;
    size_t msg_bytes = 0;
    unsigned char *dst[EK_MS_MAX_WORLD] = {};
    uint32_t *dflag[EK_MS_MAX_WORLD] = {};
    const unsigned char *src = nullptr;
    const uint32_t *sflag = nullptr;
    int32_t two_phase = 0;
};
void ek_launch_ms_chain(const EkRound &r, EkMsState *ms, const EkMsXchg &x,
                        hipStream_t s);
void ek_launch_ms_plan(const EkRound &r, EkMsState *ms, const EkMsXchg &x, float *D,
                       hipStream_t s);

void ek_launch_prepare_tiles(const float *src_aos, int64_t count, int A,
                             float *tiles, double *G, int64_t first_frame,
                             int64_t n_total, float *aos_copy, hipStream_t s);
void ek_launch_prepare_centers(const float *src_aos, int32_t count, int A,
// ... 277 lines not shown
```

enspara_amd/csrc/ek_ctx.h:

```cpp
#pragma once
#include "ek_common.h"
#include "ek_pam_sparse.h"
#include "ek_pam_policy.h"

#include <stdarg.h>
#include <stdio.h>
#include <stdlib.h>
#include <string.h>

#include <algorithm>
#include <condition_variable>
#include <mutex>
#include <new>
#include <thread>
#include <vector>

void ek_msm_scratch_free(void *w);

#define EK_N_FORMS 5

int ek_set_error(int code, const char *fmt, ...);
#define ek_fail ek_set_error

#define EK_HIP(call)                                                           \
// ... 136 lines not shown
    void invalidate() { ready = false; }
    void begin()
    {
        invalidate();
        wait.begin();
    }
};

struct ek_ctx {
    int device = 0;
    int64_t n = 0;
    int32_t A = 0;
    int64_t goff = 0;
    int64_t n_tiles = 0;
    hipStream_t stream = nullptr;
    bool own_stream = false;
    bool loaded = false;

    float *tiles = nullptr;
    float *qtiles = nullptr;
    bool qt_valid = false;
    bool no_qtiles = false;
    float *aos = nullptr;
    double *G = nullptr;
    float *dist = nullptr;
    int32_t *assign = nullptr;
    float *scratch = nullptr;
    unsigned char *rec = nullptr;
    unsigned char *rec_tmp = nullptr;
    EkBlockMax *blockmax = nullptr;
    int blockmax_cap = 0;
    EkHist *hist = nullptr;
    int32_t hist_cap = 0;
    EkCtl *ctl = nullptr;

    float *stage[2] = {nullptr, nullptr};
    float *pin[2] = {nullptr, nullptr};
    hipEvent_t up_ev[2] = {nullptr, nullptr};
    bool up_busy[2] = {false, false};
    EkCopyPool *pool = nullptr;
    int64_t stage_frames = 0;
    float *cen_aos = nullptr;
    double *cen_G = nullptr;
    int32_t cen_cap = 0;
    float *cen_tiles = nullptr;
    int32_t cen_tiles_cap = 0;
    int assign_variant = 0;
    float *cen_blocks = nullptr;
    size_t cen_blocks_cap = 0;

    float *ndist = nullptr;
    int32_t *nassign = nullptr;
    uint32_t *amb = nullptr;
    unsigned long long *amb_best = nullptr;
    unsigned int *amb_count = nullptr;
    int32_t *blockcnt = nullptr;
    int64_t *scan = nullptr;
    int64_t *sel = nullptr;
    double *sq_part = nullptr;
    EkPwShape *pw_shapes = nullptr;
    int pw_n_full = 0, pw_leaves = 0, pw_chunks = 0;
    bool pw_tail_ok = false;
    double *sq_out = nullptr;
    float *med_aos = nullptr;
    double *med_G = nullptr;
    int64_t *med_idx = nullptr;
    float *ambt = nullptr;
    double *ambG = nullptr;
    int64_t ambt_cap = 0;
    int32_t med_K = 0, med_cap = 0;
    int32_t pam_cid = -1;
    int64_t pam_frame = -1;
    int32_t *bat_blockcnt = nullptr;
    int64_t *bat_scan = nullptr;
    int64_t *bat_sel = nullptr;
    EkPamCounts cnt;
    float *pam_vecs = nullptr;
    float *pam_dprop = nullptr;
    int64_t *sel_host = nullptr;
    int64_t *cnt_host = nullptr;
    int64_t *js_host = nullptr;
    int pam_zero_copy = 1;
    int pam_bounds = 1;
    unsigned char *pam_recs = nullptr;
    EkPlan *pam_plan = nullptr;
    unsigned int *moved = nullptr;
    EkPamPrefetch pf;
    EkPamOut *pam_out_dev = nullptr;
    EkPamOut *pam_out_host = nullptr;
    EkPamWin *pam_win_dev = nullptr;
    EkPamWin *pam_win_host = nullptr;
    int32_t *med_list = nullptr;
    float *dtab = nullptr;
    EkPamTables tab;
    unsigned int *act_n_host = nullptr;
    int prune = 1;
    bool state_exact = true;
    int64_t *tmp_idx = nullptr;
    int64_t tmp_idx_cap = 0;
    int pam_sparse = 1;
    int64_t sp_max_pairs = EK_SP_MAX_PAIRS;
    int sp_exact = 0;
    EkPamOneWg sp;
    uint32_t *act_list = nullptr;
    unsigned char *sp_buf = nullptr;
    int pam_spec = 1;
    unsigned long long *sp_marks = nullptr;
    hipEvent_t win_ev = nullptr;

    int cands = -1;
    unsigned char *recsT = nullptr;
    EkPlan *plan = nullptr;
    float *vecs = nullptr;
    EkMaxHdr *hdr = nullptr;
    EkBlockMax *pm = nullptr;
    EkBlockMax *fm = nullptr;
    int fine_pick = 1;
    int pass_sweep = 1;
    int ms_two_phase = 1;
    int pick_cap = 0;
    unsigned char *top = nullptr;
    float *planD = nullptr;
    int fused = 1;
    int tri = 0;
    float *ti_D = nullptr;
    int32_t ti_cap = 0;
    uint8_t *ti_skip = nullptr;
    unsigned long long *ti_stats = nullptr;
    int64_t ti_tiles = 0, ti_skipped = 0;
    float *ti_rtab = nullptr;
    int32_t ti_rtab_cap = 0;
    uint32_t *ti_tmask = nullptr;
    float *ti_tab = nullptr;
    double *ti_tabG = nullptr;
    int32_t ti_tab_cap = 0;
    int32_t ti_tab_n = 0;
    EkPend *pend = nullptr;
    EkChainOrd *ord = nullptr;
    EkChainRow *rows = nullptr;
    uint32_t *vmask = nullptr;
    struct Guard { const char *name; unsigned char *at; };
    std::vector<Guard> guards;
    unsigned int *tick = nullptr;
    float *ctile = nullptr;
    double *ctrace = nullptr;
    int chain = 1;
    int64_t n_pad = 0;
    int32_t last_passes = 0;
    int adapt = 1;
    int64_t st_rounds[EK_N_FORMS] = {0, 0, 0, 0, 0};
    int64_t st_centers[EK_N_FORMS] = {0, 0, 0, 0, 0};
    int64_t last_form[6] = {0, 0, 0, 0, 0, 0};
    hipEvent_t evb0 = nullptr, evb1 = nullptr;

    int active_view = 1;
    int view_rho = 750;
    int view_ratio = 800;
    bool view_nomem = false;
    int64_t view_cap = 0;
    float *v_aos = nullptr, *v_tiles = nullptr, *v_qtiles = nullptr;
    double *v_G = nullptr;
    float *v_dist = nullptr;
    int32_t *v_assign = nullptr;
    uint32_t *v_act = nullptr;
    uint32_t *v_blockcnt = nullptr, *v_blockoff = nullptr;
    uint32_t *v_count = nullptr;
    int64_t view_stats[4] = {0, 0, 0, 0};

    EkMsState *ms = nullptr;
    unsigned char *ms_mbox = nullptr;
    uint32_t *ms_flags = nullptr;
    EkMsXchg ms_x;
    int ms_peers = 0;
    std::vector<void *> ms_ipc;
    int ms_T = 0;
    int ms_small = 0;
    hipEvent_t ms_ev[4] = {nullptr, nullptr, nullptr, nullptr};
    double ms_t[3] = {0.0, 0.0, 0.0};
    int64_t ms_t_n = 0;
    EkMsState ms_last;

    void *msm_scratch = nullptr;

    int fpl = 0;
    int nt = -1;
    std::vector<hipEvent_t> samp_ev;
    std::vector<int> samp_form;
    int samp_dom = 0;
    int samp_every = 0;
    int samp_used = 0;
    int64_t samp_count = 0;
    hipEvent_t ev0 = nullptr, ev1 = nullptr;
    float last_ms = 0.f;
    int32_t last_launches = 0;
};


hipError_t ek_wait(ek_ctx *c);
int ek_pick_fpl(const ek_ctx *c);
int ek_pick_nt(const ek_ctx *c);
int ek_pick_cands(const ek_ctx *c, bool wide = false, bool group = false);
int ek_ensure_qtiles(ek_ctx *c);
size_t ek_cblocks16_bytes(int32_t K, int A);
void ek_launch_cblocks16(const float *cen_aos, int32_t K, int A, float *cblocks,
                         hipStream_t s);
void ek_launch_assign16(const float *qtiles, const double *G, int64_t n, int A,
                        const float *cblocks, const double *Gc, int32_t K, float *dist,
                        int32_t *assign, hipStream_t s);
void ek_launch_pam_setup_dev(const float *aos, const double *G, int A,
                             const int64_t *frames_dev, int count, int64_t global_offset,
                             unsigned char *recs, float *ctile, double *ctrace,
                             EkPlan *plan, unsigned int *counter, hipStream_t s,
                             const float *dist, float *dprop);
extern int ek_pam_pairs_form;
int ek_form_slot(int T);
int ek_spec_alloc(ek_ctx *c);
bool ek_poison();
hipError_t ek_uncached_alloc(int device, void **ptr, size_t bytes);
void ek_uncached_free(int device, void *ptr);
#define EK_GUARD_BYTES 4096
int ek_ensure_hist(ek_ctx *c, int32_t label);
void ek_pam_forget(ek_ctx *c);
int ek_upload_centers(ek_ctx *c, const float *xyz, int32_t K);
int ek_free_all(ek_ctx *c);
hipError_t ek_malloc_named(ek_ctx *c, void **ptr, size_t bytes, const char *name);
void ek_view_free(ek_ctx *c);
void ek_round_of(ek_ctx *c, int T, double cutoff, EkRound &R);
```

enspara_amd/csrc/ek_run_policy.h:

```cpp
#pragma once
#include <algorithm>
#include <cmath>
#include <cstdint>

struct EkWait {
    int left = 0, next, first, most;
    constexpr EkWait(int first_, int most_) : next(first_), first(first_), most(most_) {}
    void lose()
    {
        left = next;
        next = std::min(2 * next, most);
    }
    void reset() { next = first; }
    bool tick()
    {
        if (left <= 0)
            return false;
        --left;
        return true;
    }
};

struct EkPickCap {
    int cap;
    bool adaptive;
    bool probing = false;
    EkWait wait{2, 64};
    int form = 0;
    double yield_home = 0.0;
    explicit EkPickCap(int option) : cap(option > 0 ? option : 4), adaptive(option <= 0) {}
    void update(int T, int32_t got, int32_t ran, int32_t room)
    {
        if (!adaptive || ran <= 0)
            return;
        const double yield = (double)got / ((double)ran * T);
        if (probing) {
            probing = false;
            if (T == form && yield > yield_home + 0.1) {
                wait.reset();
            } else {
                cap = cap == 4 ? 16 : 4;
                wait.lose();
            }
        } else if (!wait.tick() && yield < 0.65 && room > 4 * T) {
            yield_home = yield;
            form = T;
            cap = cap == 4 ? 16 : 4;
            probing = true;
        }
    }
};

inline double ek_per_round_guess(int T) { return 0.6 * T; }

struct EkFormLadder {
    int ladder[4], n = 0;
    bool adaptive;
    int home = 0;
    int form;
    bool probing = false;
    int probe_up = 1;
    double rate_home = 0.0;
    int32_t gap = 8;
    int32_t since = 0;
    EkFormLadder(bool adaptive_, bool tri, int Tmax) : adaptive(adaptive_)
    {
        if (adaptive || (tri && Tmax <= 1))
            ladder[n++] = 1;
        if (Tmax > 1) {
            if (adaptive && Tmax >= 16)
                ladder[n++] = 8;
            ladder[n++] = Tmax;
        }
        form = ladder[0];
    }
    int32_t due(int32_t left) const { return adaptive ? std::max(gap - since, 1) : left; }
    void update(int32_t got, double ms, double per_round)
    {
        if (!adaptive)
            return;
        const double rate = got / std::max(ms, 1e-6);
        if (probing) {
            probing = false;
            since = 0;
            if (rate > rate_home) {
                for (int q = 0; q < n; ++q)
                    if (ladder[q] == form)
                        home = q;
                rate_home = rate;
                gap = 8;
            } else {
                form = ladder[home];
                gap = std::min(gap * 2, 1024);
            }
            return;
        }
        rate_home = rate;
        since += got;
        if (since < gap)
            return;
        const bool up = up_ok(per_round), down = down_ok(per_round);
        int target = -1;
        if (up && down)
            target = probe_up ? home + 1 : home - 1;
        else if (up)
            target = home + 1;
        else if (down)
            target = home - 1;
        if (target >= 0) {
            probe_up = target > home ? 0 : 1;
            form = ladder[target];
            probing = true;
        } else {
            since = 0;
        }
    }
    bool up_ok(double per_round) const
    {
        const int T = ladder[home];
        return home + 1 < n && (T == 1 || per_round >= 0.8 * T);
    }
    bool down_ok(double per_round) const
    {
        if (home <= 0)
            return false;
        if (ladder[home - 1] == 1)
            return per_round < 1.8;
        return per_round < 1.35 * ladder[home - 1];
    }
};

struct EkGroupLadder {
    bool on;
    int Tmax;
    double up16, down16;
    EkWait wait16{1, 64}, wait32{1, 64};
    EkGroupLadder(bool on_, int Tmax_, bool small_shards)
        : on(on_), Tmax(Tmax_), up16(small_shards ? 4.5 : 6.5),
          down16(small_shards ? 5.5 : 8.5)
    {
    }
    int first() const { return on ? 8 : Tmax; }
    int update(int T, double per_round, int32_t ran)
    {
        if (!on || ran <= 0)
            return T;
        int want = T;
        if (T == 8) {
            if (!wait16.tick() && per_round >= up16)
                want = 16;
        } else if (T == 16) {
            if (per_round < down16) {
                want = 8;
                wait16.lose();
            } else {
                wait16.reset();
                if (!wait32.tick() && Tmax == 32 && per_round >= 14.0)
                    want = 32;
            }
        } else if (per_round < 22.0) {
            want = 16;
            wait32.lose();
        } else {
            wait32.reset();
        }
        return want;
    }
};

struct EkTriPause {
    EkWait wait{2, 64};
    unsigned long long seen[2] = {0, 0};
    bool paused() const { return wait.left > 0; }
    void look(const unsigned long long now[2])
    {
        const unsigned long long looked = now[0] - seen[0], left_out = now[1] - seen[1];
        seen[0] = now[0];
        seen[1] = now[1];
        if (looked > 0 && left_out * 50 < looked)
            wait.lose();
        else
            wait.reset();
    }
    void skipped() { (void)wait.tick(); }
};

static constexpr int EK_VIEW_MIN_ROUNDS = 24;
static constexpr int EK_VIEW_BATCH = 16;
static constexpr double EK_VIEW_IDLE = 0.95;
static constexpr int EK_VIEW_PAUSE_MAX = 8;
static constexpr int EK_VIEW_PAUSED_BATCH = 4 * EK_VIEW_BATCH;
static constexpr double EK_VIEW_REL = 1e-3, EK_VIEW_ABS = 1e-3;

struct EkViewPlan {
    float theta = 0.f;
    double guard = 0.0;
    int64_t est = 0;
    bool build = false;
};

struct EkViewPolicy {
    EkWait pause{1, EK_VIEW_PAUSE_MAX};
    EkViewPlan decide(float last_max, double rho, double shrink, const uint32_t cnt[2],
                      int64_t view_n, int64_t n, int32_t left, double per_round, bool forced)
    {
        EkViewPlan p;
        const double th = (rho * (double)last_max - EK_VIEW_ABS) / (2.0 * (1.0 + EK_VIEW_REL));
        p.theta = (float)th;
        if ((double)p.theta > th)
            p.theta = std::nextafterf(p.theta, 0.f);
        if (!(p.theta > 0.f))
            return p;
        p.guard = 2.0 * (double)p.theta * (1.0 + EK_VIEW_REL) + EK_VIEW_ABS;
        p.est = (int64_t)cnt[0] +
                (view_n > 0 ? std::max<int64_t>(0, (int64_t)cnt[1] - view_n) : 0);
        const int64_t store_n = view_n > 0 ? view_n : n;
        p.build = forced ? p.est < n
                         : ((double)p.est <= shrink * (double)store_n &&
                            (double)left >= EK_VIEW_MIN_ROUNDS * std::max(per_round, 1.0));
        if (!forced) {
            if ((double)p.est > EK_VIEW_IDLE * (double)store_n)
                pause.lose();
            else if (p.build || (double)p.est <= shrink * (double)store_n)
                pause.reset();
        }
        return p;
    }
};

inline int32_t ek_batch_single(int form, int32_t left, int32_t due, double per_round,
                               bool probing, bool forced, int view)
{
    const bool one = form == 1;
    int32_t batch;
    if (one)
        batch = std::min(left, probing ? 4 : std::min(due, 256));
    else if (probing)
        batch = 3;
    else
        batch = std::max(2, std::min(256, (int32_t)(std::min(left, due) / per_round) + 1));
    if (forced)
        batch = std::min(batch, 2);
    else if (view && !one)
        batch = std::min(batch, view == 2 ? EK_VIEW_PAUSED_BATCH : EK_VIEW_BATCH);
    return batch;
}

#ifndef EK_MS_BATCH8
#define EK_MS_BATCH8 12
#endif
inline int32_t ek_batch_group(int T, int32_t left, double per_round, bool ladder)
{
    int32_t batch = std::max(2, std::min(256, (int32_t)(left / per_round) + 2));
    if (ladder)
        batch = std::min(batch, T == 8 ? EK_MS_BATCH8 : (T == 16 ? 64 : 48));
    return batch;
}
```

enspara_amd/csrc/ek_view.h:

```cpp
#pragma once
#include "ek_common.h"

#define EK_VIEW_SEL 1024

static inline size_t ek_view_sel_blocks(int64_t n)
{
    return (size_t)((n + EK_VIEW_SEL - 1) / EK_VIEW_SEL);
}
void ek_launch_view_select(const float *dist, int64_t n, float theta, uint32_t *blockcnt,
                           uint32_t *blockoff, uint32_t *act, int64_t act_cap,
                           uint32_t *count, hipStream_t s);
void ek_launch_view_gather(const uint32_t *act, int64_t n_v, int A, const float *aos,
                           const double *G, const float *dist, const int32_t *assign,
                           float *aos_v, float *tiles_v, double *G_v, float *dist_v,
                           int32_t *assign_v, hipStream_t s);
void ek_launch_view_build(const uint32_t *act, int64_t n_v, int A, bool quad, const float *aos,
                          const double *G, const float *dist, const int32_t *assign,
                          float *aos_v, float *out_v, double *G_v, float *dist_v,
                          int32_t *assign_v, hipStream_t s);
void ek_launch_view_tiles(const float *qtiles, int64_t n_tiles, int A, float *tiles,
                          hipStream_t s);
void ek_launch_view_look(const float *dist, int64_t n, const EkCtl *ctl, double rho, double rel,
                         double abs_, uint32_t *count, hipStream_t s);
void ek_launch_view_diff(const void *a, const void *b, size_t words,
                         unsigned long long *count, hipStream_t s);
void ek_launch_view_scatter(const uint32_t *act, int64_t n_v, const float *dist_v,
                            const int32_t *assign_v, float *dist, int32_t *assign,
                            EkHist *hist, int32_t label_lo, int32_t label_cap,
                            const EkCtl *ctl, int64_t goff, hipStream_t s);
```

enspara_amd/csrc/ek_view.hip:

```cpp
#include <algorithm>
#include "ek_view.h"

#define EK_VIEW_FPT (EK_VIEW_SEL / EK_BLOCK)
static_assert(EK_VIEW_FPT == 4, "a thread reads its frames' distances as one float4");

static __device__ __forceinline__ bool ek_view_active(float d, float theta)
{
    return !(d <= theta);
}

static __device__ __forceinline__ unsigned ek_view_flags(const float *__restrict__ dist,
                                                         int64_t f0, int64_t n, float theta)
{
    unsigned m = 0;
    if (f0 + EK_VIEW_FPT <= n) {
        const float4 t = *(const float4 *)(dist + f0);
        m = (ek_view_active(t.x, theta) ? 1u : 0u) | (ek_view_active(t.y, theta) ? 2u : 0u) |
            (ek_view_active(t.z, theta) ? 4u : 0u) | (ek_view_active(t.w, theta) ? 8u : 0u);
    } else {
        for (int q = 0; q < EK_VIEW_FPT; ++q)
            if (f0 + q < n && ek_view_active(dist[f0 + q], theta))
                m |= 1u << q;
    }
    return m;
}

static __device__ __forceinline__ unsigned ek_view_block_scan(unsigned v, unsigned *red,
                                                              unsigned *total)
{
    const int tid = threadIdx.x, lane = tid & (EK_WAVE - 1), wave = tid / EK_WAVE;
    unsigned inc = v;
#pragma unroll
    for (int off = 1; off < EK_WAVE; off <<= 1) {
        const unsigned o = (unsigned)__shfl_up((int)inc, off, EK_WAVE);
        if (lane >= off)
            inc += o;
    }
    if (lane == EK_WAVE - 1)
        red[wave] = inc;
    __syncthreads();
    unsigned before = 0, sum = 0;
#pragma unroll
    for (int w = 0; w < EK_BLOCK / EK_WAVE; ++w) {
        if (w < wave)
            before += red[w];
        sum += red[w];
    }
    __syncthreads();
    *total = sum;
    return before + inc - v;
}

__global__ void __launch_bounds__(EK_BLOCK)
ek_view_count_kernel(const float *__restrict__ dist, int64_t n, float theta,
                     uint32_t *__restrict__ blockcnt)
{
    __shared__ unsigned red[EK_BLOCK / EK_WAVE];
    const int64_t f0 = ((int64_t)blockIdx.x * EK_BLOCK + threadIdx.x) * EK_VIEW_FPT;
    const unsigned m = f0 < n ? ek_view_flags(dist, f0, n, theta) : 0u;
    unsigned total;
    (void)ek_view_block_scan((unsigned)__popc(m), red, &total);
    if (threadIdx.x == 0)
        blockcnt[blockIdx.x] = total;
}

__global__ void __launch_bounds__(EK_BLOCK)
ek_view_scan_kernel(const uint32_t *__restrict__ blockcnt, int nblk,
                    uint32_t *__restrict__ blockoff, uint32_t *__restrict__ count)
{
    __shared__ unsigned red[EK_BLOCK / EK_WAVE];
    const int per = (nblk + EK_BLOCK - 1) / EK_BLOCK;
    const int lo = threadIdx.x * per, hi = lo + per < nblk ? lo + per : nblk;
    unsigned mine = 0;
    for (int b = lo; b < hi; ++b)
        mine += blockcnt[b];
    unsigned total;
    unsigned run = ek_view_block_scan(mine, red, &total);
    if (blockoff)
        for (int b = lo; b < hi; ++b) {
            blockoff[b] = run;
            run += blockcnt[b];
        }
    if (threadIdx.x == 0)
        count[0] = total;
}

__global__ void __launch_bounds__(EK_BLOCK)
ek_view_write_kernel(const float *__restrict__ dist, int64_t n, float theta,
                     const uint32_t *__restrict__ blockoff, uint32_t *__restrict__ act,
                     int64_t act_cap)
{
    __shared__ unsigned red[EK_BLOCK / EK_WAVE];
    const int64_t f0 = ((int64_t)blockIdx.x * EK_BLOCK + threadIdx.x) * EK_VIEW_FPT;
    const unsigned m = f0 < n ? ek_view_flags(dist, f0, n, theta) : 0u;
    unsigned total;
    unsigned p = blockoff[blockIdx.x] + ek_view_block_scan((unsigned)__popc(m), red, &total);
#pragma unroll
    for (int q = 0; q < EK_VIEW_FPT; ++q)
        if ((m >> q) & 1u) {
            if (p < act_cap)
                act[p] = (uint32_t)(f0 + q);
            ++p;
        }
}

void ek_launch_view_select(const float *dist, int64_t n, float theta, uint32_t *blockcnt,
                           uint32_t *blockoff, uint32_t *act, int64_t act_cap,
                           uint32_t *count, hipStream_t s)
{
    if (n <= 0) {
        (void)hipMemsetAsync(count, 0, sizeof(uint32_t), s);
        return;
    }
    const unsigned nblk = (unsigned)ek_view_sel_blocks(n);
    hipLaunchKernelGGL(ek_view_count_kernel, dim3(nblk), dim3(EK_BLOCK), 0, s, dist, n,
                       theta, blockcnt);
    hipLaunchKernelGGL(ek_view_scan_kernel, dim3(1), dim3(EK_BLOCK), 0, s, blockcnt,
                       (int)nblk, act ? blockoff : (uint32_t *)nullptr, count);
    if (act)
        hipLaunchKernelGGL(ek_view_write_kernel, dim3(nblk), dim3(EK_BLOCK), 0, s, dist, n,
                           theta, blockoff, act, act_cap);
}

#define EK_VIEW_CH 16
#define EK_VIEW_ROWF (3 * EK_VIEW_CH + 1)

__global__ void __launch_bounds__(EK_BLOCK)
ek_view_gather_kernel(const uint32_t *__restrict__ act, int64_t n_v, int A,
                      const float *__restrict__ aos, const double *__restrict__ G,
                      const float *__restrict__ dist, const int32_t *__restrict__ assign,
                      float *__restrict__ aos_v, float *__restrict__ tiles_v,
                      double *__restrict__ G_v, float *__restrict__ dist_v,
                      int32_t *__restrict__ assign_v)
{
    static_assert(EK_BLOCK == EK_TILE, "one workgroup per tile of the view");
    __shared__ float stage[EK_BLOCK * EK_VIEW_ROWF];
    __shared__ uint32_t src[EK_BLOCK];
    const int t = threadIdx.x;
    const int64_t p0 = (int64_t)blockIdx.x * EK_TILE;
    const int64_t p = p0 + t;
    const bool live = p < n_v;
    const int rows_here = (int)((n_v - p0 < EK_TILE) ? (n_v - p0) : EK_TILE);
    const uint32_t f = live ? act[p] : 0u;
    src[t] = f;
    if (live) {
        G_v[p] = G[f];
        dist_v[p] = dist[f];
        assign_v[p] = assign[f];
    }
    __syncthreads();
    const size_t A3 = (size_t)3 * A;
    float *tile = tiles_v + (size_t)blockIdx.x * A3 * EK_TILE + t;
    for (int a0 = 0; a0 < A; a0 += EK_VIEW_CH) {
        const int w = 3 * ((A - a0 < EK_VIEW_CH) ? (A - a0) : EK_VIEW_CH);
// ... 50 lines not shown
    constexpr int SWEEPS = EK_VIEW_BROWS / RPS;
    __shared__ float stage[EK_VIEW_BROWS * EK_VIEW_BROWF];
    __shared__ uint32_t src[EK_VIEW_BROWS];
    const int t = threadIdx.x;
    const size_t tile = blockIdx.x >> 2;
    const int qw = blockIdx.x & 3;
    const int64_t p0 = (int64_t)tile * EK_TILE + EK_VIEW_BROWS * qw;
    const int rows_here =
        (int)(n_v - p0 >= EK_VIEW_BROWS ? EK_VIEW_BROWS : (n_v > p0 ? n_v - p0 : 0));
    if (t < EK_VIEW_BROWS) {
        const int64_t p = p0 + t;
        const uint32_t f = t < rows_here ? act[p] : 0u;
        src[t] = f;
        if (t < rows_here) {
            G_v[p] = G[f];
            dist_v[p] = dist[f];
            assign_v[p] = assign[f];
        }
    }
    __syncthreads();
    const size_t A3 = (size_t)3 * A;
    const int NQ = (A + 3) / 4;
    const int jl = t & (LPR - 1), r0 = t / LPR;
    const int slot = t & 63, wv = t >> 6, qe = slot >> 4, qf = slot & 15;
    for (int a0 = 0; a0 < A; a0 += EK_VIEW_BCH) {
        const int w = 3 * ((A - a0 < EK_VIEW_BCH) ? (A - a0) : EK_VIEW_BCH);
        const int we = w / VEC;
        vec_t v[SWEEPS][3];
#pragma unroll
        for (int it = 0; it < SWEEPS; ++it) {
            const int r = r0 + it * RPS;
            const vec_t *s = (const vec_t *)(aos + (size_t)src[r] * A3 + 3 * a0);
#pragma unroll
            for (int m = 0; m < 3; ++m) {
                const int j = jl + m * LPR;
                if (r < rows_here && j < we)
                    v[it][m] = s[j];
            }
        }
#pragma unroll
        for (int it = 0; it < SWEEPS; ++it) {
            const int r = r0 + it * RPS;
            vec_t *d = (vec_t *)(aos_v + (size_t)(p0 + r) * A3 + 3 * a0);
            float *st = stage + r * EK_VIEW_BROWF;
#pragma unroll
            for (int m = 0; m < 3; ++m) {
                const int j = jl + m * LPR;
                if (r < rows_here && j < we) {
                    d[j] = v[it][m];
                    if constexpr (VEC == 4) {
#pragma unroll
                        for (int x = 0; x < 4; ++x)
                            st[4 * j + x] = v[it][m][x];
                    } else {
                        st[j] = v[it][m];
                    }
                }
            }
        }
        __syncthreads();
        if constexpr (QUAD) {
            ek_view_v4f *dst = (ek_view_v4f *)out_v + tile * (size_t)NQ * 3 * EK_TILE +
                               EK_VIEW_BROWS * qw + slot;
            for (int qq = wv; qq < EK_VIEW_BCH / 4; qq += EK_BLOCK / EK_WAVE) {
                const int q = a0 / 4 + qq;
                if (q >= NQ)
                    break;
                const bool atom = 4 * q + qe < A;
#pragma unroll
                for (int k = 0; k < 3; ++k) {
                    ek_view_v4f o;
#pragma unroll
                    for (int g = 0; g < 4; ++g) {
                        const int fr = 16 * g + qf;
                        o[g] = (atom && fr < rows_here)
                                   ? stage[fr * EK_VIEW_BROWF + 3 * (4 * qq + qe) + k] : 0.f;
                    }
                    dst[(size_t)(q * 3 + k) * EK_TILE] = o;
                }
            }
        } else {
            float *tp = out_v + tile * A3 * EK_TILE + EK_VIEW_BROWS * qw + slot;
            const float *row = stage + slot * EK_VIEW_BROWF;
            for (int j = wv; j < w; j += EK_BLOCK / EK_WAVE)
                tp[(size_t)(3 * a0 + j) * EK_TILE] = slot < rows_here ? row[j] : 0.f;
        }
        __syncthreads();
    }
}

void ek_launch_view_build(const uint32_t *act, int64_t n_v, int A, bool quad, const float *aos,
                          const double *G, const float *dist, const int32_t *assign,
                          float *aos_v, float *out_v, double *G_v, float *dist_v,
                          int32_t *assign_v, hipStream_t s)
{
    if (n_v <= 0)
        return;
    const unsigned tiles = (unsigned)((n_v + EK_TILE - 1) / EK_TILE);
#define EK_VIEW_BUILD(VEC, QUAD)                                                          \
    hipLaunchKernelGGL((ek_view_build_kernel<VEC, QUAD>), dim3(4 * tiles), dim3(EK_BLOCK), 0, \
                       s, act, n_v, A, aos, G, dist, assign, aos_v, out_v, G_v, dist_v,   \
                       assign_v)
    if (A % 4 == 0) {
        if (quad)
            EK_VIEW_BUILD(4, true);
        else
            EK_VIEW_BUILD(4, false);
    } else {
        if (quad)
            EK_VIEW_BUILD(1, true);
        else
            EK_VIEW_BUILD(1, false);
    }
#undef EK_VIEW_BUILD
}

__global__ void __launch_bounds__(EK_BLOCK)
ek_view_tiles_kernel(const float *__restrict__ qtiles, int A, int NQ,
                     float *__restrict__ tiles)
{
    const int l = threadIdx.x;
    const int w = l >> 6, e = (l >> 4) & 3, f16 = l & 15;
    const size_t tile = blockIdx.x;
    const ek_view_v4f *src = (const ek_view_v4f *)qtiles + tile * (size_t)NQ * 3 * EK_TILE + l;
    float *dst = tiles + tile * 3 * (size_t)A * EK_TILE + 64 * w + f16;
    for (int q = blockIdx.y; q < NQ; q += gridDim.y) {
        const int a = 4 * q + e;
        if (a >= A)
            continue;
#pragma unroll
        for (int k = 0; k < 3; ++k) {
            const ek_view_v4f v = src[(size_t)(q * 3 + k) * EK_TILE];
#pragma unroll
            for (int g = 0; g < 4; ++g)
                dst[(size_t)(3 * a + k) * EK_TILE + 16 * g] = v[g];
        }
    }
}

void ek_launch_view_tiles(const float *qtiles, int64_t n_tiles, int A, float *tiles,
                          hipStream_t s)
{
    if (n_tiles <= 0)
        return;
    const int NQ = (A + 3) / 4;
    const unsigned gy = (unsigned)std::max<int64_t>(
        1, std::min<int64_t>(NQ, 2048 / std::max<int64_t>(n_tiles, 1)));
    hipLaunchKernelGGL(ek_view_tiles_kernel, dim3((unsigned)n_tiles, gy), dim3(EK_BLOCK), 0, s,
                       qtiles, A, NQ, tiles);
}

#define EK_VIEW_LOOK_SEL (8 * EK_VIEW_SEL)
__global__ void __launch_bounds__(EK_BLOCK)
ek_view_look_kernel(const float *__restrict__ dist, int64_t n, const EkCtl *__restrict__ ctl,
                    double rho, double rel, double abs_, uint32_t *__restrict__ count)
{
    __shared__ unsigned red[EK_BLOCK / EK_WAVE];
    const double th = (rho * (double)ctl->last_max - abs_) / (2.0 * (1.0 + rel));
    float theta = (float)th;
    if ((double)theta > th && theta > 0.f)
        theta = __uint_as_float(__float_as_uint(theta) - 1u);
    unsigned mine = 0;
#pragma unroll
    for (int q = 0; q < EK_VIEW_LOOK_SEL / EK_VIEW_SEL; ++q) {
        const int64_t f0 = (((int64_t)blockIdx.x * (EK_VIEW_LOOK_SEL / EK_VIEW_SEL) + q) *
                                EK_BLOCK + threadIdx.x) * EK_VIEW_FPT;
        mine += f0 < n ? (unsigned)__popc(ek_view_flags(dist, f0, n, theta)) : 0u;
    }
    unsigned total;
    (void)ek_view_block_scan(mine, red, &total);
    if (threadIdx.x == 0 && total)
        atomicAdd(count, total);
}

void ek_launch_view_look(const float *dist, int64_t n, const EkCtl *ctl, double rho, double rel,
                         double abs_, uint32_t *count, hipStream_t s)
{
    if (n <= 0)
        return;
    hipLaunchKernelGGL(ek_view_look_kernel,
                       dim3((unsigned)((n + EK_VIEW_LOOK_SEL - 1) / EK_VIEW_LOOK_SEL)),
                       dim3(EK_BLOCK), 0, s, dist, n, ctl, rho, rel, abs_, count);
}

__global__ void __launch_bounds__(EK_BLOCK)
ek_view_diff_kernel(const uint32_t *__restrict__ a, const uint32_t *__restrict__ b, size_t n,
                    unsigned long long *__restrict__ count)
{
    unsigned mine = 0;
    for (size_t i = (size_t)blockIdx.x * EK_BLOCK + threadIdx.x; i < n;
         i += (size_t)gridDim.x * EK_BLOCK)
        mine += a[i] != b[i] ? 1u : 0u;
    if (mine)
        atomicAdd(count, (unsigned long long)mine);
}

void ek_launch_view_diff(const void *a, const void *b, size_t words,
                         unsigned long long *count, hipStream_t s)
{
    if (words == 0)
        return;
    const unsigned blocks =
        (unsigned)std::min<size_t>((words + EK_BLOCK - 1) / EK_BLOCK, (size_t)4096);
    hipLaunchKernelGGL(ek_view_diff_kernel, dim3(blocks), dim3(EK_BLOCK), 0, s,
                       (const uint32_t *)a, (const uint32_t *)b, words, count);
}

__global__ void __launch_bounds__(EK_BLOCK)
ek_view_scatter_kernel(const uint32_t *__restrict__ act, int64_t n_v,
                       const float *__restrict__ dist_v,
                       const int32_t *__restrict__ assign_v, float *__restrict__ dist,
                       int32_t *__restrict__ assign, EkHist *__restrict__ hist,
                       int32_t label_lo, int32_t label_cap, const EkCtl *__restrict__ ctl,
                       int64_t goff)
{
    const int64_t p = (int64_t)blockIdx.x * EK_BLOCK + threadIdx.x;
    if (p < n_v) {
        const uint32_t f = act[p];
        dist[f] = dist_v[p];
        assign[f] = assign_v[p];
    }
    int32_t hi = ctl->n_done;
    if (hi > label_cap)
        hi = label_cap;
    for (int64_t l = label_lo + p; l < hi; l += (int64_t)gridDim.x * EK_BLOCK) {
        const int64_t q = hist[l].gidx - goff;
        if (hist[l].set && q >= 0 && q < n_v)
            hist[l].gidx = goff + (int64_t)act[q];
    }
}

void ek_launch_view_scatter(const uint32_t *act, int64_t n_v, const float *dist_v,
                            const int32_t *assign_v, float *dist, int32_t *assign,
                            EkHist *hist, int32_t label_lo, int32_t label_cap,
                            const EkCtl *ctl, int64_t goff, hipStream_t s)
{
    if (n_v <= 0)
        return;
    hipLaunchKernelGGL(ek_view_scatter_kernel,
                       dim3((unsigned)((n_v + EK_BLOCK - 1) / EK_BLOCK)), dim3(EK_BLOCK), 0,
                       s, act, n_v, dist_v, assign_v, dist, assign, hist, label_lo,
                       label_cap, ctl, goff);
}
```

enspara_amd/device.py:

```python
import ctypes as C

import numpy as np

from . import _lib
from .exception import DataInvalid


def as_xyz(X):
    if hasattr(X, "xyz"):
        X = X.xyz
    elif hasattr(X, "_data") and hasattr(X, "lengths"):
        X = X._data
    X = np.asarray(X)
    if X.ndim == 2 and X.shape[1] == 3:
        X = X[None]
    if X.ndim != 3 or X.shape[2] != 3:
        raise DataInvalid(
            "RMSD clustering needs coordinates shaped (n_frames, n_atoms, 3); "
            "got %s" % (X.shape,))
    return np.ascontiguousarray(X, dtype=np.float32)


def _option_key(key):
    if isinstance(key, str):
# ... 309 lines not shown
                                          C.c_void_p(int(recs_out_ptr))))

    def spec_round(self, recs_all_ptr, n_recs, dist_cutoff):
        _lib.check(self.lib.ek_spec_round(
            self._h, C.c_void_p(int(recs_all_ptr)), int(n_recs),
            float(dist_cutoff)))

    def spec_localmax(self, hdr_out_ptr):
        _lib.check(self.lib.ek_spec_localmax(self._h,
                                             C.c_void_p(int(hdr_out_ptr))))

    def spec_apply(self, hdrs_all_ptr, n_hdrs, dist_cutoff):
        _lib.check(self.lib.ek_spec_apply(
            self._h, C.c_void_p(int(hdrs_all_ptr)), int(n_hdrs),
            float(dist_cutoff)))

    def spec_chain_bytes(self):
        a, b = C.c_int32(), C.c_int32()
        _lib.check(self.lib.ek_spec_chain_bytes(C.byref(a), C.byref(b)))
        return a.value, b.value

    def spec_chain_rows(self, rows_out_ptr):
        _lib.check(self.lib.ek_spec_chain_rows(
            self._h, C.c_void_p(int(rows_out_ptr))))

    def spec_chain_max(self, rows_all_ptr, n_shards, hdrs_out_ptr):
        _lib.check(self.lib.ek_spec_chain_max(
            self._h, C.c_void_p(int(rows_all_ptr)), int(n_shards),
            C.c_void_p(int(hdrs_out_ptr))))

    def spec_chain_apply(self, hdrs_all_ptr, n_shards, dist_cutoff):
        _lib.check(self.lib.ek_spec_chain_apply(
            self._h, C.c_void_p(int(hdrs_all_ptr)), int(n_shards),
            float(dist_cutoff)))

    def spec_round_end(self, recs_out_ptr):
        _lib.check(self.lib.ek_spec_round_end(self._h,
                                              C.c_void_p(int(recs_out_ptr))))

    def spec_progress(self):
        nd, st = C.c_int32(), C.c_int32()
        _lib.check(self.lib.ek_spec_progress(self._h, C.byref(nd),
                                             C.byref(st)))
        return nd.value, bool(st.value)

    def spec_rounds(self):
        r = C.c_int32()
        _lib.check(self.lib.ek_spec_rounds(self._h, C.byref(r)))
        return r.value

    def msm_counts(self, lengths, lag_time, n_states, sliding_window=True):
        lengths = np.ascontiguousarray(lengths, dtype=np.int64)
        for name, v in (("lag_time", lag_time), ("n_states", n_states)):
            if not 1 <= int(v) < 2 ** 31:
                raise DataInvalid("%s=%d is outside [1, 2^31)" % (name, int(v)))
        cap = max(1, min(int(self.n), int(n_states) * int(n_states)))
        rows = np.empty(cap, dtype=np.int32)
        cols = np.empty(cap, dtype=np.int32)
        vals = np.empty(cap, dtype=np.int64)
        nnz = C.c_int64()
        _lib.check(self.lib.ek_msm_counts_ctx(
            self._h, _lib.i64p(lengths), len(lengths), int(lag_time),
            1 if sliding_window else 0, int(n_states), cap, _lib.i32p(rows),
            _lib.i32p(cols), _lib.i64p(vals), C.byref(nnz)))
        k = nnz.value
        return rows[:k], cols[:k], vals[:k]

    def ms_setup(self, world, rank):
        b = C.c_size_t()
        _lib.check(self.lib.ek_ms_setup(self._h, int(world), int(rank),
                                        C.byref(b)))
        return b.value

    def ms_mailbox(self, ipc=False):
        if ipc:
            hm = C.create_string_buffer(64)
            hf = C.create_string_buffer(64)
            _lib.check(self.lib.ek_ms_mailbox(self._h, None, None, hm, hf))
            return hm.raw, hf.raw
        m, f = C.c_void_p(), C.c_void_p()
        _lib.check(self.lib.ek_ms_mailbox(self._h, C.byref(m), C.byref(f), None,
                                          None))
        return m.value, f.value

    def ms_connect(self, peer, mbox=None, flags=None, ipc=None):
        if ipc is not None:
            hm = C.create_string_buffer(bytes(ipc[0]), 64)
            hf = C.create_string_buffer(bytes(ipc[1]), 64)
            _lib.check(self.lib.ek_ms_connect(self._h, int(peer), None, None,
                                              hm, hf))
        else:
            _lib.check(self.lib.ek_ms_connect(
                self._h, int(peer), C.c_void_p(mbox), C.c_void_p(flags), None,
                None))

    def ms_begin(self, first_label, limit):
        _lib.check(self.lib.ek_ms_begin(self._h, int(first_label), int(limit)))

    def ms_local(self, dist_cutoff, message_out_ptr):
        _lib.check(self.lib.ek_ms_local(self._h, float(dist_cutoff),
                                        C.c_void_p(int(message_out_ptr))))

    def ms_global(self, dist_cutoff, messages_all_ptr):
        _lib.check(self.lib.ek_ms_global(self._h, float(dist_cutoff),
                                         C.c_void_p(int(messages_all_ptr))))

    def ms_end(self):
        _lib.check(self.lib.ek_ms_end(self._h))

    def ms_state(self):
        m, e, r = C.c_int32(), C.c_int32(), C.c_int32()
        _lib.check(self.lib.ek_ms_state(self._h, C.byref(m), C.byref(e),
                                        C.byref(r)))
        return m.value, e.value, r.value

    def reserve_centers(self, n_centers):
        _lib.check(self.lib.ek_reserve_centers(self._h, int(n_centers)))

    def debug_guards(self):
        rc = int(self.lib.ek_debug_guards(self._h))
        if rc < 0:
            _lib.check(rc)
        return rc

    def ms_run(self, first_label, max_new, dist_cutoff):
        max_new = int(max_new)
        idx = np.empty(max(max_new, 1), dtype=np.int64)
        cd = np.empty(max(max_new, 1), dtype=np.float32)
        n_added = C.c_int32()
        fmax = C.c_float()
        _lib.check(self.lib.ek_ms_run(
            self._h, int(first_label), max_new, float(dist_cutoff),
            C.byref(n_added), _lib.i64p(idx), _lib.f32p(cd), C.byref(fmax)))
        k = n_added.value
        return idx[:k].copy(), cd[:k].copy(), fmax.value

    def run_stats(self):
        p = np.zeros(5, dtype=np.int64)
        k = np.zeros(5, dtype=np.int64)
        _lib.check(self.lib.ek_run_stats(self._h, _lib.i64p(p), _lib.i64p(k)))
        return {T: (int(p[i]), int(k[i])) for i, T in enumerate((1, 4, 8, 16, 32))}

    def ti_stats(self):
        t, k = C.c_int64(), C.c_int64()
        _lib.check(self.lib.ek_ti_stats(self._h, C.byref(t), C.byref(k)))
        return t.value, k.value

    def view_stats(self):
        s = np.zeros(4, dtype=np.int64)
        _lib.check(self.lib.ek_view_stats(self._h, _lib.i64p(s)))
        return {"views": int(s[0]), "streamed": int(s[1]), "left_out": int(s[2]),
                "guard_exits": int(s[3])}

    def last_run_form(self):
        s = np.zeros(6, dtype=np.int64)
        _lib.check(self.lib.ek_last_run_form(self._h, _lib.i64p(s)))
        return {"frames_per_lane": int(s[0]), "nontemporal": int(s[1]),
                "sweep_in_pass": int(s[2]), "fine_pick": int(s[3]),
                "coarse_entries": int(s[4]), "pick_entries": int(s[5])}

    def view_layout_check(self, theta):
        out = np.zeros(4, dtype=np.int64)
        _lib.check(self.lib.ek_view_layout_check(self._h, float(theta), _lib.i64p(out)))
        return tuple(int(v) for v in out)

    def history(self, first, count):
        idx = np.empty(max(count, 1), dtype=np.int64)
        cd = np.empty(max(count, 1), dtype=np.float32)
        nd = C.c_int32()
        _lib.check(self.lib.ek_history_download(
            self._h, int(first), int(count), _lib.i64p(idx), _lib.f32p(cd),
            C.byref(nd)))
        return idx[:count], cd[:count], nd.value

    def reset_history(self):
        _lib.check(self.lib.ek_history_reset(self._h))

    def set_frames_per_lane(self, fpl):
        _lib.check(self.lib.ek_set_frames_per_lane(self._h, int(fpl)))

    def set_option(self, key, value):
        _lib.check(self.lib.ek_set_option(self._h, _option_key(key), int(value)))

    def get_option(self, key):
        v = C.c_int32()
        _lib.check(self.lib.ek_get_option(self._h, _option_key(key), C.byref(v)))
        return v.value

    def last_run_timing(self):
        ms = C.c_float()
        k = C.c_int32()
        _lib.check(self.lib.ek_last_run_timing(self._h, C.byref(ms),
                                               C.byref(k)))
        return ms.value, k.value

    def timing_begin(self, sample_every=32, max_samples=512):
        _lib.check(self.lib.ek_timing_begin(self._h, int(sample_every),
                                            int(max_samples)))

    def timing_end(self):
        ms = C.c_float()
        k = C.c_int32()
        _lib.check(self.lib.ek_timing_end(self._h, C.byref(ms), C.byref(k)))
        return ms.value, k.value

    def timing_form(self):
        t = C.c_int32()
        _lib.check(self.lib.ek_timing_form(self._h, C.byref(t)))
        return t.value
```

include/enspara_hip.h:

```cpp
#ifndef ENSPARA_HIP_H
#define ENSPARA_HIP_H

#include <stddef.h>
#include <stdint.h>

#ifdef __cplusplus
extern "C" {
#endif

#define EK_ABI_VERSION 1
#define EK_TILE 256

#define EK_OK 0
#define EK_EARG (-1)
#define EK_EHIP (-2)
#define EK_ESTATE (-3)
#define EK_ENOMEM (-4)

typedef struct ek_ctx ek_ctx;

int ek_abi_version(void);
const char *ek_last_error(void);
int ek_device_count(void);

int ek_ctx_create(int device, int64_t n_frames, int32_t n_atoms,
                  int64_t global_offset, void *stream, ek_ctx **out);
int ek_ctx_destroy(ek_ctx *ctx);
int ek_ctx_sync(ek_ctx *ctx);
void *ek_ctx_stream(ek_ctx *ctx);

int ek_load_frames(ek_ctx *ctx, const float *xyz, int64_t first,
                   int64_t count, int src_is_device);

int ek_rmsd_to_center(ek_ctx *ctx, int64_t frame_index,
                      const float *center_xyz, float *out_host);

int ek_state_reset(ek_ctx *ctx);
int ek_state_download(ek_ctx *ctx, float *dist_host, int32_t *assign_host);
int ek_state_upload(ek_ctx *ctx, const float *dist_host,
                    const int32_t *assign_host);

size_t ek_record_bytes(int32_t n_atoms);
int ek_local_candidate(ek_ctx *ctx, void *rec_dev);
void *ek_own_record(ek_ctx *ctx);

int ek_kcenters_step(ek_ctx *ctx, const void *recs_dev, int32_t n_recs,
                     int32_t label, double dist_cutoff, void *own_rec_out);

int ek_kcenters_run(ek_ctx *ctx, int32_t first_label, int32_t max_new,
                    double dist_cutoff, int32_t *n_added,
                    int64_t *center_index_out, float *center_dist_out,
                    float *final_maxdist);

int ek_spec_candidates(ek_ctx *ctx);
int ek_round_candidates(ek_ctx *ctx);
int ek_quad_copy_ready(ek_ctx *ctx);
int ek_spec_begin(ek_ctx *ctx, int32_t first_label, int32_t limit,
                  void *recs_out);
int ek_spec_round(ek_ctx *ctx, const void *recs_all, int32_t n_recs,
                  double dist_cutoff);
int ek_spec_localmax(ek_ctx *ctx, void *hdr_out);
int ek_spec_apply(ek_ctx *ctx, const void *hdrs_all, int32_t n_hdrs,
                  double dist_cutoff);
int ek_spec_round_end(ek_ctx *ctx, void *recs_out);
int ek_spec_progress(ek_ctx *ctx, int32_t *n_done, int32_t *stopped);
int ek_spec_chain_bytes(int32_t *rows_bytes, int32_t *hdrs_bytes);
int ek_spec_chain_rows(ek_ctx *ctx, void *rows_out);
int ek_spec_chain_max(ek_ctx *ctx, const void *rows_all, int32_t n_shards,
                      void *hdrs_out);
int ek_spec_chain_apply(ek_ctx *ctx, const void *hdrs_all, int32_t n_shards,
                        double dist_cutoff);
int ek_ms_setup(ek_ctx *ctx, int32_t world, int32_t rank, size_t *message_bytes);
int ek_ms_mailbox(ek_ctx *ctx, void **mbox, void **flags, void *ipc_mbox,
                  void *ipc_flags);
int ek_ms_connect(ek_ctx *ctx, int32_t peer, void *mbox, void *flags,
                  const void *ipc_mbox, const void *ipc_flags);
int ek_reserve_centers(ek_ctx *ctx, int32_t n_centers);
int ek_ms_begin(ek_ctx *ctx, int32_t first_label, int32_t limit);
int ek_ms_local(ek_ctx *ctx, double dist_cutoff, void *message_out);
int ek_ms_global(ek_ctx *ctx, double dist_cutoff, const void *messages_all);
int ek_ms_end(ek_ctx *ctx);
int ek_ms_diag(ek_ctx *ctx, int64_t *counts, double *ms);
int ek_ms_state(ek_ctx *ctx, int32_t *mode, int32_t *exchanges, int32_t *err);
int ek_ms_run(ek_ctx *ctx, int32_t first_label, int32_t max_new,
              double dist_cutoff, int32_t *n_added, int64_t *center_index_out,
              float *center_dist_out, float *final_maxdist);
int ek_spec_rounds(ek_ctx *ctx, int32_t *rounds);
int ek_run_stats(ek_ctx *ctx, int64_t *passes, int64_t *centers);
int ek_ti_stats(ek_ctx *ctx, int64_t *tiles, int64_t *skipped);
int ek_view_stats(ek_ctx *ctx, int64_t *stats);
int ek_last_run_form(ek_ctx *ctx, int64_t *out);
int ek_view_layout_check(ek_ctx *ctx, float theta, int64_t *out);

int ek_history_download(ek_ctx *ctx, int32_t first, int32_t count,
                        int64_t *center_index_out, float *center_dist_out,
                        int32_t *n_done);
int ek_history_reset(ek_ctx *ctx);

int ek_assign_nearest(ek_ctx *ctx, const float *centers_xyz,
                      int32_t n_centers);

int ek_pam_begin(ek_ctx *ctx, const int64_t *medoid_frames, int32_t n_medoids);
int ek_pam_count_members(ek_ctx *ctx, int32_t cid, int64_t *count);
int ek_pam_select_member(ek_ctx *ctx, int32_t cid, int64_t j,
                         int64_t *frame_index);
int ek_pam_propose(ek_ctx *ctx, int32_t cid, int64_t frame_index,
                   double *old_cost, double *new_cost, int64_t *n_ambiguous);
int ek_pam_propose_member(ek_ctx *ctx, int32_t cid, int64_t j,
                          int64_t *frame_index, double *old_cost,
                          double *new_cost, int64_t *n_ambiguous);
int ek_pam_commit(ek_ctx *ctx, int accept);

int ek_pam_count_members_batch(ek_ctx *ctx, int32_t cid0, int32_t count,
                               int64_t *counts);
int ek_pam_select_members_batch(ek_ctx *ctx, int32_t cid0, int32_t count,
                                const int64_t *js, int64_t *frames);
int ek_pam_prefetch(ek_ctx *ctx, const int64_t *frames, int32_t count);
int ek_pam_prefetch_window(ek_ctx *ctx, const int64_t *frames, int32_t count,
                           int32_t win_lo, int32_t win_count);
int ek_pam_prefetch_passes(ek_ctx *ctx, int64_t *restricted, int64_t *full);
int ek_pam_propose_ex(ek_ctx *ctx, int32_t cid, int64_t frame_index,
                      int64_t n_members, int32_t win_lo, int32_t win_count,
                      double *old_cost, double *new_cost, int64_t *n_ambiguous,
                      uint32_t *moved_mask);
int ek_pam_prefetch_stats(ek_ctx *ctx, int64_t *hits, int64_t *misses);
int ek_pam_sparse_stats(ek_ctx *ctx, int64_t *windows, int64_t *ended_early);
int ek_pam_ahead_stats(ek_ctx *ctx, int64_t *slots_taken_over);
int32_t ek_pam_window_max(void);
int ek_pam_window_run(ek_ctx *ctx, int32_t cid0, int32_t count,
                      const int64_t *frames, const int64_t *n_members,
                      int32_t win_lo, int32_t win_count, int32_t *n_done,
                      int32_t *accept, double *old_cost, double *new_cost,
                      int64_t *n_ambiguous);

int64_t ek_np_choice_draws(const uint32_t *raw, int64_t n_raw, int64_t *pos,
                           const int64_t *m, int64_t count, int64_t *out);
int ek_pam_sweep(ek_ctx *ctx, int32_t n_medoids, int32_t width, const uint32_t *raw,
                 int64_t n_raw, int64_t *pos, const int64_t *proposals, int32_t *cid,
                 int64_t *medoids, int32_t *accept, double *old_cost,
                 double *new_cost, int64_t *n_ambiguous, int32_t *status);

int ek_centered_frames(ek_ctx *ctx, const int64_t *local_frames,
                       const int32_t *rows, int32_t count, float *aos_dev,
                       double *G_dev);
int ek_pam_begin_table(ek_ctx *ctx, const float *aos_dev, const double *G_dev,
                       int32_t n_medoids);
int ek_pam_prefetch_centers(ek_ctx *ctx, const float *aos_dev,
                            const double *G_dev, int32_t count);
int ek_pam_prefetch_centers_window(ek_ctx *ctx, const float *aos_dev,
                                   const double *G_dev, int32_t count,
                                   int32_t win_lo, int32_t win_count);
int ek_pam_propose_center(ek_ctx *ctx, int32_t cid, int32_t slot,
                          const float *center_aos_dev,
                          const double *center_G_dev, int64_t n_members_local,
                          int32_t win_lo, int32_t win_count, void *out_dev);

int ek_msm_counts(int device, const int32_t *assigns, const int64_t *lengths,
                  int64_t n_trj, int32_t lag_time, int32_t sliding_window,
                  int32_t n_states, int64_t capacity, int32_t *rows_out,
                  int32_t *cols_out, int64_t *counts_out, int64_t *nnz_out);
int ek_msm_counts_ctx(ek_ctx *ctx, const int64_t *lengths, int64_t n_trj,
                      int32_t lag_time, int32_t sliding_window, int32_t n_states,
                      int64_t capacity, int32_t *rows_out, int32_t *cols_out,
                      int64_t *counts_out, int64_t *nnz_out);
int ek_msm_row_normalize(int device, const int64_t *indptr, const double *data,
                         int64_t n_rows, double *probs_out, double *rowsum_out);
int ek_msm_mle_prinz(int device, int32_t n, int64_t n_pairs, int32_t n_levels,
                     const int64_t *level_ptr, const int32_t *pair_i,
                     const int32_t *pair_j, const double *c_ij,
                     const double *c_ji, const double *c_diag,
                     const double *c_rs, double *x_pairs, double *x_diag,
                     double *x_rs, double tol, int64_t max_iter,
                     int64_t *n_iter_out, double *logl_out);
int ek_msm_bace_prune(int device, int32_t n, const double *c, const double *w,
                      float *d_out);
int ek_msm_bace_run(int device, int32_t n, const double *c, const double *w,
                    const int32_t *kept, int32_t n_kept, int32_t n_macrostates,
                    int32_t n_merges, void *records_out, int32_t dmat_steps,
                    float *dmat_out);

int ek_lu_solve(int device, int32_t n, const double *A, int32_t nrhs, const double *B,
                double *X, int32_t *pivots_out, int32_t *info_out);
int ek_lu_set_timing(int on);
int ek_lu_last_timing(double *ms_out, double *gemm_flops_out);
int ek_tpt_committors(int device, int32_t n, const double *T, const int32_t *sources,
                      int32_t n_sources, const int32_t *sinks, int32_t n_sinks,
                      double *q_out, int32_t *info_out);
int ek_tpt_mfpts_sinks(int device, int32_t n, const double *T, const int32_t *sinks,
                       int32_t n_sinks, double lagtime, double *t_out,
                       int32_t *info_out);
int ek_tpt_mfpts_all(int device, int32_t n, const double *T, const double *pops,
                     double lagtime, double *mfpt_out, int32_t *info_out);
int ek_tpt_fluxes(int device, int32_t n, const double *T, const int32_t *sources,
                  int32_t n_sources, const int32_t *sinks, int32_t n_sinks,
                  const double *pops, int32_t net, double *q_out, double *flux_out,
                  int32_t *info_out);

typedef struct ek_mi ek_mi;
int ek_mi_open(int device, int32_t fx, int32_t fy, int32_t nx, int32_t ny, ek_mi **out);
int ek_mi_add(ek_mi *h, const uint8_t *X, const uint8_t *Y, int64_t frames);
int ek_mi_load_counts(ek_mi *h, const uint32_t *jc, uint64_t n_obs);
int ek_mi_counts(ek_mi *h, uint32_t *jc_out);
int ek_mi_information(ek_mi *h, double *mi_out);
int ek_mi_last_timing(ek_mi *h, double *ms_out);
int ek_mi_close(ek_mi *h);

typedef struct ek_cards ek_cards;
int ek_cards_open(int device, int32_t f, int32_t n_states, ek_cards **out);
int ek_cards_add(ek_cards *h, const uint8_t *X, int64_t frames);
int ek_cards_stats(ek_cards *h, int64_t *stats_out);
int ek_cards_disorder(ek_cards *h, const int64_t *lo, const int64_t *hi);
int ek_cards_disorder_codes(ek_cards *h, int32_t traj, uint8_t *out);
int ek_cards_matrices(ek_cards *h, double *mi_out);
int ek_cards_counts(ek_cards *h, int32_t which, uint32_t *jc_out);
int ek_cards_last_timing(ek_cards *h, double *ms_out);
int ek_cards_close(ek_cards *h);
int ek_cards_scan_chunk(void);

typedef struct ek_sasa ek_sasa;
int ek_sasa_open(int device, int32_t atoms, const float *R, int32_t n_points,
                 const float *points, int32_t n_groups, const int32_t *group_offsets,
                 const int32_t *group_atoms, ek_sasa **out);
int ek_sasa_run(ek_sasa *h, const float *xyz, int64_t frames, int64_t chunk_frames,
                int32_t *counts_out, float *areas_out, float *groups_out);
int ek_sasa_last_timing(ek_sasa *h, double *ms_out);
int ek_sasa_close(ek_sasa *h);

typedef struct ek_rmsf ek_rmsf;
int ek_rmsf_open(int device, int32_t atoms, int32_t n_sel, const int32_t *sel,
                 const float *reference, int32_t n_groups, const int32_t *group_offsets,
                 const int32_t *group_atoms, ek_rmsf **out);
int ek_rmsf_run(ek_rmsf *h, const float *xyz, int64_t frames, const double *weights,
                int64_t ref_index, int64_t chunk_frames, float *aligned_out,
                double *rotations_out, float *rmsd_out, uint32_t *flags_out);
int ek_rmsf_fetch(ek_rmsf *h, double *atom_sums_out, double *group_sums_out);
int ek_rmsf_last_timing(ek_rmsf *h, double *ms_out);
int ek_rmsf_close(ek_rmsf *h);

typedef struct ek_msm_boot ek_msm_boot;
int ek_msm_boot_open(int device, const int32_t *assigns, const int64_t *lengths,
                     int64_t n_units, int32_t lag_time, int32_t sliding_window,
                     int32_t n_states, int64_t nnz, const int64_t *indptr,
                     const int32_t *cols, int32_t n_trials, const int32_t *mult,
// ... 262 lines not shown
```

Before: 23.18 billion.

## Merge control, look counts and tile stats into one device block; rework ladder batching

Packs the control struct, view-look counters and triangle-inequality tile stats into a single device control block. This lets each batch read everything back with one device-to-host copy. The two view-look launches become one kernel that finalizes its own counts with a last-arriver atomic, which removes a memset and a separate copy per look. The form-ladder policy gains a windowed rate estimate and a 'calm' state that stretches batch lengths when no probe is warranted, so fewer host round trips happen per center. Host loop counters are added for diagnostics. The risk is that longer batches delay adaptation or waste rounds.

New measurement: 23.25 billion (median of 6 runs). No clear change (+0.3%).

```diff
diff --git a/enspara_amd/_lib.py b/enspara_amd/_lib.py
--- a/enspara_amd/_lib.py
+++ b/enspara_amd/_lib.py
@@ -24,7 +24,7 @@
     "ek_spec_apply", "ek_spec_round_end", "ek_spec_progress", "ek_spec_rounds",
     "ek_spec_chain_bytes", "ek_spec_chain_rows", "ek_spec_chain_max",
     "ek_spec_chain_apply", "ek_run_stats", "ek_ti_stats", "ek_view_stats",
-    "ek_last_run_form",
+    "ek_last_run_form", "ek_run_loop_stats",
     "ek_view_layout_check",
     "ek_ms_setup", "ek_ms_mailbox", "ek_ms_connect", "ek_ms_begin", "ek_ms_local",
     "ek_ms_global", "ek_ms_end", "ek_ms_run", "ek_ms_state", "ek_ms_diag",
@@ -198,6 +198,7 @@
     L.ek_ti_stats.argtypes = [vp, i64p, i64p]
     L.ek_view_stats.argtypes = [vp, i64p]
     L.ek_last_run_form.argtypes = [vp, i64p]
+    L.ek_run_loop_stats.argtypes = [vp, i64p]
     L.ek_view_layout_check.argtypes = [vp, f32, i64p]
     L.ek_assign_nearest.argtypes = [vp, f32p, i32]
     f64p = C.POINTER(C.c_double)
diff --git a/enspara_amd/csrc/ek_api.hip b/enspara_amd/csrc/ek_api.hip
--- a/enspara_amd/csrc/ek_api.hip
+++ b/enspara_amd/csrc/ek_api.hip
@@ -301,7 +301,7 @@
     (void)ek_dev_free(c->ti_tab);
     (void)ek_dev_free(c->ti_tabG);
     (void)ek_dev_free(c->ti_skip);
-    (void)ek_dev_free(c->ti_stats);
+    c->ti_stats = nullptr;
     (void)ek_dev_free(c->pend);
     (void)ek_dev_free(c->ord);
     (void)ek_dev_free(c->tick);
@@ -407,7 +407,7 @@
     EK_ALLOC(c->rec_tmp, recb);
     EK_ALLOC(c->blockmax, (size_t)c->blockmax_cap * sizeof(EkBlockMax));
     EK_ALLOC(c->hist, (size_t)c->hist_cap * sizeof(EkHist));
-    EK_ALLOC(c->ctl, sizeof(EkCtl));
+    EK_ALLOC(c->ctl, sizeof(EkCtlBlock));
     EK_ALLOC(c->recsT, recb * EK_MAX_CANDS);
     EK_ALLOC(c->plan, sizeof(EkPlan));
     EK_ALLOC(c->hdr, sizeof(EkMaxHdr));
@@ -436,7 +436,9 @@
         e = hipMemsetAsync(c->hist, 0, (size_t)c->hist_cap * sizeof(EkHist),
                            c->stream);
     if (e == hipSuccess)
-        e = hipMemsetAsync(c->ctl, 0, sizeof(EkCtl), c->stream);
+        e = hipMemsetAsync(c->ctl, 0, sizeof(EkCtlBlock), c->stream);
+    if (e == hipSuccess)
+        c->ti_stats = ((EkCtlBlock *)c->ctl)->ti_stats;
     if (e == hipSuccess)
         e = hipMemsetAsync(c->rec, 0, recb, c->stream);
     if (e == hipSuccess)
@@ -990,11 +992,6 @@
             if (!c->ti_skip)
                 EK_HIP(ek_dev_malloc((void **)&c->ti_skip,
                                      (size_t)std::max<int64_t>(c->n_tiles, 1)));
-            if (!c->ti_stats) {
-                EK_HIP(ek_dev_malloc((void **)&c->ti_stats, 2 * sizeof(unsigned long long)));
-                EK_HIP(hipMemsetAsync(c->ti_stats, 0, 2 * sizeof(unsigned long long),
-                                      c->stream));
-            }
             if (label == 0)
                 EK_HIP(hipMemsetAsync(c->ti_stats, 0, 2 * sizeof(unsigned long long),
                                       c->stream));
diff --git a/enspara_amd/csrc/ek_api_run.hip b/enspara_amd/csrc/ek_api_run.hip
--- a/enspara_amd/csrc/ek_api_run.hip
+++ b/enspara_amd/csrc/ek_api_run.hip
@@ -179,17 +179,23 @@
     bool pending = false;
     bool masks_fresh = false;
     bool looked = false;
-    uint32_t look_cnt[2] = {0, 0};
-    EkCtl cr;
+    EkCtlBlock back;
+    EkCtl &cr = back.ctl;
     double per_round;
     int32_t rounds_before = 0;
     EkRun(ek_ctx *c_, EkViewRun &view_, bool adaptive, bool tri_, int Tmax)
         : c(c_), view(view_), tri(tri_), lad(adaptive, tri_, Tmax), cap(c_->pick_cap),
           per_round(ek_per_round_guess(lad.form))
     {
-        memset(&cr, 0, sizeof(cr));
+        memset(&back, 0, sizeof(back));
     }
 };
+
+static hipError_t ek_run_wait(ek_ctx *c)
+{
+    c->loop_stats[ek_ctx::LS_WAITS]++;
+    return ek_wait(c);
+}
 
 static int ek_run_reserve_tri(ek_ctx *c, int32_t goal)
 {
@@ -204,8 +210,6 @@
     if (!c->ti_skip)
         EK_HIP(ek_dev_malloc((void **)&c->ti_skip,
                              (size_t)std::max<int64_t>(c->n_tiles, 1)));
-    if (!c->ti_stats)
-        EK_HIP(ek_dev_malloc((void **)&c->ti_stats, 2 * sizeof(unsigned long long)));
     EK_HIP(hipMemsetAsync(c->ti_stats, 0, 2 * sizeof(unsigned long long),
                           c->stream));
     if (goal > c->ti_rtab_cap) {
@@ -250,6 +254,7 @@
     R.sweep = (run.fused && (c->pass_sweep == 2 ||
                              (c->pass_sweep == 1 && ek_sweep_pays(R.n)))) ? 1 : 0;
     R.cutoff = the_view ? std::max(run.dist_cutoff, run.view.guard) : run.dist_cutoff;
+    run.lad.store_changed();
 }
 
 static void ek_run_leave_view(EkRun &run)
@@ -268,7 +273,7 @@
     EkViewRun &view = run.view;
     run.looked = false;
     const EkViewPlan p =
-        run.vp.decide(run.cr.last_max, run.rho, run.shrink, run.look_cnt,
+        run.vp.decide(run.cr.last_max, run.rho, run.shrink, run.back.look,
                       view.on ? view.n : 0, c->n, left, run.per_round, run.forced);
     if (!p.build)
         return EK_OK;
@@ -283,7 +288,7 @@
                           c->view_cap, c->v_count, c->stream);
     EK_CHECK_LAUNCH();
     EK_HIP(hipMemcpyAsync(&nv, c->v_count, sizeof(nv), hipMemcpyDeviceToHost, c->stream));
-    EK_HIP(ek_wait(c));
+    EK_HIP(ek_run_wait(c));
     if (nv > 0 && (int64_t)nv < c->n && (int64_t)nv <= c->view_cap) {
         view.n = nv;
         view.label_lo = run.cr.n_done;
@@ -336,6 +341,7 @@
     if (form != 1)
         run.per_round = ek_per_round_guess(form);
     run.held = form;
+    c->loop_stats[ek_ctx::LS_BOOT]++;
     return EK_OK;
 }
 
@@ -459,16 +465,11 @@
         run.view_mode = 0;
         return EK_OK;
     }
-    EK_HIP(hipMemsetAsync(c->v_count, 0, sizeof(run.look_cnt), c->stream));
-    ek_launch_view_look(run.R.dist, run.R.n, c->ctl, run.rho, EK_VIEW_REL, EK_VIEW_ABS,
-                        c->v_count, c->stream);
-    if (run.view.on)
-        ek_launch_view_look(c->dist, c->n, c->ctl, run.rho, EK_VIEW_REL, EK_VIEW_ABS,
-                            c->v_count + 1, c->stream);
+    ek_launch_view_look(run.R.dist, run.R.n, c->dist, run.view.on ? c->n : 0, c->ctl, run.rho,
+                        EK_VIEW_REL, EK_VIEW_ABS, c->stream);
     EK_CHECK_LAUNCH();
-    EK_HIP(hipMemcpyAsync(run.look_cnt, c->v_count, sizeof(run.look_cnt),
-                          hipMemcpyDeviceToHost, c->stream));
     run.looked = true;
+    c->loop_stats[ek_ctx::LS_LOOKS]++;
     return EK_OK;
 }
 
@@ -477,14 +478,11 @@
     ek_ctx *c = run.c;
     const bool one = form == 1, masks = run.R.tmask != nullptr;
     const int32_t before = run.cr.n_done;
-    EK_HIP(hipMemcpyAsync(&run.cr, c->ctl, sizeof(run.cr), hipMemcpyDeviceToHost, c->stream));
-    unsigned long long ti_now[2] = {0, 0};
+    EK_HIP(hipMemcpyAsync(&run.back, c->ctl, offsetof(EkCtlBlock, look_tick),
+                          hipMemcpyDeviceToHost, c->stream));
+    EK_HIP(ek_run_wait(c));
     if (masks)
-        EK_HIP(hipMemcpyAsync(ti_now, c->ti_stats, sizeof(ti_now), hipMemcpyDeviceToHost,
-                              c->stream));
-    EK_HIP(ek_wait(c));
-    if (masks)
-        run.ti.look(ti_now);
+        run.ti.look(run.back.ti_stats);
     else if (!one)
         run.ti.skipped();
     got = run.cr.n_done - before;
@@ -506,7 +504,7 @@
     const int32_t zero = 0;
     EK_HIP(hipMemcpyAsync(&c->ctl->stopped, &zero, sizeof(zero), hipMemcpyHostToDevice,
                           c->stream));
-    EK_HIP(ek_wait(c));
+    EK_HIP(ek_run_wait(c));
     run.cr.stopped = 0;
     run.held = -1;
     run.looked = false;
@@ -534,17 +532,17 @@
         run.held = form;
         EK_HIP(hipMemcpyAsync(&run.cr, c->ctl, sizeof(run.cr), hipMemcpyDeviceToHost,
                               c->stream));
-        EK_HIP(ek_wait(c));
+        EK_HIP(ek_run_wait(c));
     }
     if (run.tri) {
         unsigned long long st[2] = {0, 0};
         EK_HIP(hipMemcpyAsync(st, c->ti_stats, sizeof(st), hipMemcpyDeviceToHost, c->stream));
-        EK_HIP(ek_wait(c));
+        EK_HIP(ek_run_wait(c));
         c->ti_tiles = (int64_t)st[0];
         c->ti_skipped = (int64_t)st[1];
     }
     EK_HIP(hipEventRecord(c->ev1, c->stream));
-    EK_HIP(ek_wait(c));
+    EK_HIP(ek_run_wait(c));
     EK_HIP(hipEventElapsedTime(&c->last_ms, c->ev0, c->ev1));
     if (run.held == 1) {
         ek_launch_blockmax(c->dist, c->n, c->blockmax, c->stream);
@@ -553,7 +551,7 @@
     if (run.held >= 0)
         EK_HIP(hipMemcpyAsync(c->rec, c->recsT, ek_rec_bytes(c->A), hipMemcpyDeviceToDevice,
                               c->stream));
-    EK_HIP(ek_wait(c));
+    EK_HIP(ek_run_wait(c));
     const int32_t added_t =
         std::min(max_new, std::max(0, run.cr.n_done - run.first_label));
     const int64_t passes = c->st_rounds[0] + c->st_rounds[1] + c->st_rounds[2] +
@@ -585,9 +583,11 @@
     memset(&ctlw, 0, sizeof(ctlw));
     ctlw.n_done = first_label;
     ctlw.limit = goal;
+    for (int k = 0; k < ek_ctx::LS_N; ++k)
+        c->loop_stats[k] = 0;
     EK_HIP(hipMemcpyAsync(c->ctl, &ctlw, sizeof(ctlw), hipMemcpyHostToDevice,
                           c->stream));
-    EK_HIP(ek_wait(c));
+    EK_HIP(ek_run_wait(c));
     for (int m = 0; m < EK_N_FORMS; ++m)
         c->st_rounds[m] = c->st_centers[m] = 0;
     c->view_stats[0] = c->view_stats[1] = c->view_stats[2] = c->view_stats[3] = 0;
@@ -630,15 +630,15 @@
     EK_HIP(hipEventRecord(c->ev0, c->stream));
     while (run.cr.n_done < goal) {
         const int32_t left = goal - run.cr.n_done;
+        if (run.view_mode && run.looked && std::isfinite(run.cr.last_max))
+            EK_RC(ek_run_enter_view(run, left));
+        run.looked = false;
         const int form = run.lad.form;
         const bool one = form == 1;
         R.T = form;
         const bool masks = tri && fused && form >= 4 && !run.ti.paused();
         R.tmask = masks ? c->ti_tmask : nullptr;
         R.pick_cap = run.cap.cap;
-        if (run.view_mode && run.looked && std::isfinite(run.cr.last_max))
-            EK_RC(ek_run_enter_view(run, left));
-        run.looked = false;
         if (view.on && !view.tiles_valid && form < 16) {
             ek_launch_view_tiles(c->v_qtiles, R.n_pad / EK_TILE, c->A, c->v_tiles, c->stream);
             EK_CHECK_LAUNCH();
@@ -648,7 +648,11 @@
             EK_RC(ek_run_bootstrap(run, form));
         const int32_t batch =
             ek_batch_single(form, left, run.lad.due(left), run.per_round, run.lad.probing,
-                            run.forced, !run.view_mode ? 0 : (run.vp.pause.left > 0 ? 2 : 1));
+                            run.forced, !run.view_mode ? 0 : (run.vp.pause.left > 0 ? 2 : 1),
+                            run.lad.rounds_cap());
+        c->loop_stats[ek_ctx::LS_BATCHES + ek_form_slot(form)]++;
+        c->loop_stats[ek_ctx::LS_LONGEST] =
+            std::max<int64_t>(c->loop_stats[ek_ctx::LS_LONGEST], batch);
         EK_HIP(hipEventRecord(c->evb0, c->stream));
         EK_RC(ek_run_enqueue_batch(run, form, batch));
         EK_HIP(hipEventRecord(c->evb1, c->stream));
@@ -670,7 +674,14 @@
             continue;
         float bms = 0.f;
         EK_HIP(hipEventElapsedTime(&bms, c->evb0, c->evb1));
-        run.lad.update(got, bms, run.per_round);
+        const bool probed = run.lad.probing;
+        const int home = run.lad.home;
+        run.lad.batch_done(got, ran, bms);
+        if (probed && run.lad.home != home)
+            c->loop_stats[run.lad.home > home ? ek_ctx::LS_UP_WON : ek_ctx::LS_DOWN_WON]++;
+        if (run.lad.probing)
+            c->loop_stats[run.lad.form > run.lad.ladder[run.lad.home] ? ek_ctx::LS_UP
+                                                                       : ek_ctx::LS_DOWN]++;
     }
     return ek_run_finish(run, max_new, n_added, center_index_out, center_dist_out,
                          final_maxdist);
@@ -721,6 +732,8 @@
 
     ek_note_run_form(c, ek_pick_fpl(c), ek_pick_nt(c), false, 1, 0, false);
     c->view_stats[0] = c->view_stats[1] = c->view_stats[2] = c->view_stats[3] = 0;
+    for (int k = 0; k < ek_ctx::LS_N; ++k)
+        c->loop_stats[k] = 0;
     const bool open_loop = !(dist_cutoff > 0.0);
     const int32_t batch = open_loop ? max_new : 16;
     int32_t issued = 0;
@@ -861,3 +874,12 @@
         stats[k] = c->view_stats[k];
     return EK_OK;
 }
+
+extern "C" int ek_run_loop_stats(ek_ctx *c, int64_t *out)
+{
+    if (!c || !out)
+        return ek_fail(EK_EARG, "ek_run_loop_stats: NULL argument");
+    for (int k = 0; k < ek_ctx::LS_N; ++k)
+        out[k] = c->loop_stats[k];
+    return EK_OK;
+}
diff --git a/enspara_amd/csrc/ek_common.h b/enspara_amd/csrc/ek_common.h
--- a/enspara_amd/csrc/ek_common.h
+++ b/enspara_amd/csrc/ek_common.h
@@ -44,6 +44,16 @@
     int32_t n_rounds;
     int32_t pad[3];
 };
+
+struct EkCtlBlock {
+    EkCtl ctl;
+    uint32_t look[2];
+    uint32_t look_acc[2];
+    unsigned long long ti_stats[2];
+    unsigned int look_tick;
+    uint32_t pad[3];
+};
+static_assert(sizeof(EkCtl) == 32 && sizeof(EkCtlBlock) == 80, "control block layout");
 
 struct EkMaxHdr {
     float maxdist;
diff --git a/enspara_amd/csrc/ek_ctx.h b/enspara_amd/csrc/ek_ctx.h
--- a/enspara_amd/csrc/ek_ctx.h
+++ b/enspara_amd/csrc/ek_ctx.h
@@ -312,6 +312,9 @@
     int64_t st_centers[EK_N_FORMS] = {0, 0, 0, 0, 0};
     int64_t last_form[6] = {0, 0, 0, 0, 0, 0};
     hipEvent_t evb0 = nullptr, evb1 = nullptr;
+    enum { LS_WAITS = 0, LS_BATCHES = 1, LS_LONGEST = 6, LS_UP = 7, LS_UP_WON = 8, LS_DOWN = 9,
+           LS_DOWN_WON = 10, LS_BOOT = 11, LS_LOOKS = 12, LS_N = 13 };
+    int64_t loop_stats[LS_N] = {0};
 
     int active_view = 1;
     int view_rho = 750;
diff --git a/enspara_amd/csrc/ek_run_policy.h b/enspara_amd/csrc/ek_run_policy.h
--- a/enspara_amd/csrc/ek_run_policy.h
+++ b/enspara_amd/csrc/ek_run_policy.h
@@ -53,6 +53,8 @@
 
 inline double ek_per_round_guess(int T) { return 0.6 * T; }
 
+static constexpr int EK_LADDER_WINDOW = 8;
+static constexpr int EK_BATCH_MAX = 256;
 struct EkFormLadder {
     int ladder[4], n = 0;
     bool adaptive;
@@ -63,6 +65,10 @@
     double rate_home = 0.0;
     int32_t gap = 8;
     int32_t since = 0;
+    bool calm = false;
+    int32_t calm_rounds = EK_LADDER_WINDOW;
+    int win_form = 0;
+    double win_got = 0.0, win_ran = 0.0;
     EkFormLadder(bool adaptive_, bool tri, int Tmax) : adaptive(adaptive_)
     {
         if (adaptive || (tri && Tmax <= 1))
@@ -74,7 +80,69 @@
         }
         form = ladder[0];
     }
-    int32_t due(int32_t left) const { return adaptive ? std::max(gap - since, 1) : left; }
+    bool settled() const
+    {
+        return ladder[home] == 1 || (win_form == ladder[home] && win_ran >= EK_LADDER_WINDOW);
+    }
+    int32_t due(int32_t left) const
+    {
+        return adaptive && !calm && (probing || settled()) ? std::max(gap - since, 1) : left;
+    }
+    int32_t rounds_cap() const
+    {
+        if (!adaptive || probing)
+            return EK_BATCH_MAX;
+        if (!settled())
+            return std::max(1, (int32_t)std::ceil(
+                                   EK_LADDER_WINDOW - (win_form == ladder[home] ? win_ran : 0.0)));
+        return calm ? calm_rounds : EK_BATCH_MAX;
+    }
+    void store_changed()
+    {
+        rate_home = 0.0;
+        if (probing) {
+            probing = false;
+            form = ladder[home];
+        }
+    }
+    void batch_done(int32_t got, int32_t ran, double ms)
+    {
+        if (!adaptive)
+            return;
+        if (probing) {
+            const int probed = form;
+            update(got, ms, 0.0);
+            if (form == probed) {
+                win_form = probed;
+                win_got = got;
+                win_ran = std::max(ran, 0);
+            }
+            return;
+        }
+        const int T = ladder[home];
+        if (T == 1) {
+            update(got, ms, 1.0);
+            return;
+        }
+        if (win_form != T) {
+            win_form = T;
+            win_got = win_ran = 0.0;
+        }
+        if (ran >= EK_LADDER_WINDOW) {
+            win_got = got;
+            win_ran = ran;
+        } else if (ran > 0) {
+            const double keep = std::min(win_ran, (double)(EK_LADDER_WINDOW - ran));
+            win_got = got + (win_ran > 0.0 ? win_got * keep / win_ran : 0.0);
+            win_ran = ran + keep;
+        }
+        if (!settled()) {
+            rate_home = got / std::max(ms, 1e-6);
+            since += got;
+            return;
+        }
+        update(got, ms, win_got / win_ran);
+    }
     void update(int32_t got, double ms, double per_round)
     {
         if (!adaptive)
@@ -89,6 +157,8 @@
                         home = q;
                 rate_home = rate;
                 gap = 8;
+                calm = false;
+                calm_rounds = EK_LADDER_WINDOW;
             } else {
                 form = ladder[home];
                 gap = std::min(gap * 2, 1024);
@@ -97,23 +167,27 @@
         }
         rate_home = rate;
         since += got;
+        const bool up = up_ok(per_round), down = down_ok(per_round);
+        if (!up && !down) {
+            calm_rounds = calm && home + 1 >= n ? std::min(2 * calm_rounds, EK_BATCH_MAX)
+                                                : EK_LADDER_WINDOW;
+            calm = true;
+            if (since >= gap)
+                since = 0;
+            return;
+        }
+        calm = false;
+        calm_rounds = EK_LADDER_WINDOW;
         if (since < gap)
             return;
-        const bool up = up_ok(per_round), down = down_ok(per_round);
-        int target = -1;
+        int target;
         if (up && down)
             target = probe_up ? home + 1 : home - 1;
-        else if (up)
-            target = home + 1;
-        else if (down)
-            target = home - 1;
-        if (target >= 0) {
-            probe_up = target > home ? 0 : 1;
-            form = ladder[target];
-            probing = true;
-        } else {
-            since = 0;
-        }
+        else
+            target = up ? home + 1 : home - 1;
+        probe_up = target > home ? 0 : 1;
+        form = ladder[target];
+        probing = true;
     }
     bool up_ok(double per_round) const
     {
@@ -229,16 +303,18 @@
 };
 
 inline int32_t ek_batch_single(int form, int32_t left, int32_t due, double per_round,
-                               bool probing, bool forced, int view)
+                               bool probing, bool forced, int view,
+                               int32_t cap = EK_BATCH_MAX)
 {
     const bool one = form == 1;
     int32_t batch;
     if (one)
-        batch = std::min(left, probing ? 4 : std::min(due, 256));
+        batch = std::min(left, probing ? 4 : std::min(due, EK_BATCH_MAX));
     else if (probing)
         batch = 3;
     else
-        batch = std::max(2, std::min(256, (int32_t)(std::min(left, due) / per_round) + 1));
+        batch = std::max(2, std::min(std::min(cap, EK_BATCH_MAX),
+                                     (int32_t)(std::min(left, due) / per_round) + 1));
     if (forced)
         batch = std::min(batch, 2);
     else if (view && !one)
diff --git a/enspara_amd/csrc/ek_view.h b/enspara_amd/csrc/ek_view.h
--- a/enspara_amd/csrc/ek_view.h
+++ b/enspara_amd/csrc/ek_view.h
@@ -20,8 +20,8 @@
                           int32_t *assign_v, hipStream_t s);
 void ek_launch_view_tiles(const float *qtiles, int64_t n_tiles, int A, float *tiles,
                           hipStream_t s);
-void ek_launch_view_look(const float *dist, int64_t n, const EkCtl *ctl, double rho, double rel,
-                         double abs_, uint32_t *count, hipStream_t s);
+void ek_launch_view_look(const float *dist0, int64_t n0, const float *dist1, int64_t n1,
+                         EkCtl *ctl, double rho, double rel, double abs_, hipStream_t s);
 void ek_launch_view_diff(const void *a, const void *b, size_t words,
                          unsigned long long *count, hipStream_t s);
 void ek_launch_view_scatter(const uint32_t *act, int64_t n_v, const float *dist_v,
diff --git a/enspara_amd/csrc/ek_view.hip b/enspara_amd/csrc/ek_view.hip
--- a/enspara_amd/csrc/ek_view.hip
+++ b/enspara_amd/csrc/ek_view.hip
@@ -1,5 +1,6 @@
 #include <algorithm>
 #include "ek_view.h"
+#include "ek_reduce.h"
 
 #define EK_VIEW_FPT (EK_VIEW_SEL / EK_BLOCK)
 static_assert(EK_VIEW_FPT == 4, "a thread reads its frames' distances as one float4");
@@ -356,35 +357,53 @@
 
 #define EK_VIEW_LOOK_SEL (8 * EK_VIEW_SEL)
 __global__ void __launch_bounds__(EK_BLOCK)
-ek_view_look_kernel(const float *__restrict__ dist, int64_t n, const EkCtl *__restrict__ ctl,
-                    double rho, double rel, double abs_, uint32_t *__restrict__ count)
+ek_view_look_kernel(const float *__restrict__ dist0, int64_t n0, unsigned nb0,
+                    const float *__restrict__ dist1, int64_t n1, EkCtlBlock *blk, double rho,
+                    double rel, double abs_)
 {
     __shared__ unsigned red[EK_BLOCK / EK_WAVE];
-    const double th = (rho * (double)ctl->last_max - abs_) / (2.0 * (1.0 + rel));
+    const double th = (rho * (double)blk->ctl.last_max - abs_) / (2.0 * (1.0 + rel));
     float theta = (float)th;
     if ((double)theta > th && theta > 0.f)
         theta = __uint_as_float(__float_as_uint(theta) - 1u);
+    const bool own = blockIdx.x >= nb0;
+    const float *__restrict__ dist = own ? dist1 : dist0;
+    const int64_t n = own ? n1 : n0;
+    const int64_t b = own ? blockIdx.x - nb0 : blockIdx.x;
     unsigned mine = 0;
 #pragma unroll
     for (int q = 0; q < EK_VIEW_LOOK_SEL / EK_VIEW_SEL; ++q) {
-        const int64_t f0 = (((int64_t)blockIdx.x * (EK_VIEW_LOOK_SEL / EK_VIEW_SEL) + q) *
-                                EK_BLOCK + threadIdx.x) * EK_VIEW_FPT;
+        const int64_t f0 = ((b * (EK_VIEW_LOOK_SEL / EK_VIEW_SEL) + q) * EK_BLOCK +
+                            threadIdx.x) * EK_VIEW_FPT;
         mine += f0 < n ? (unsigned)__popc(ek_view_flags(dist, f0, n, theta)) : 0u;
     }
     unsigned total;
     (void)ek_view_block_scan(mine, red, &total);
     if (threadIdx.x == 0 && total)
-        atomicAdd(count, total);
-}
-
-void ek_launch_view_look(const float *dist, int64_t n, const EkCtl *ctl, double rho, double rel,
-                         double abs_, uint32_t *count, hipStream_t s)
-{
-    if (n <= 0)
-        return;
-    hipLaunchKernelGGL(ek_view_look_kernel,
-                       dim3((unsigned)((n + EK_VIEW_LOOK_SEL - 1) / EK_VIEW_LOOK_SEL)),
-                       dim3(EK_BLOCK), 0, s, dist, n, ctl, rho, rel, abs_, count);
+        (void)__hip_atomic_fetch_add(&blk->look_acc[own ? 1 : 0], total, __ATOMIC_RELAXED,
+                                     __HIP_MEMORY_SCOPE_AGENT);
+    if (!ek_arrive_last(&blk->look_tick))
+        return;
+    if (threadIdx.x < 2) {
+        blk->look[threadIdx.x] = __hip_atomic_load(&blk->look_acc[threadIdx.x], __ATOMIC_RELAXED,
+                                                   __HIP_MEMORY_SCOPE_AGENT);
+        __hip_atomic_store(&blk->look_acc[threadIdx.x], 0u, __ATOMIC_RELAXED,
+                           __HIP_MEMORY_SCOPE_AGENT);
+    }
+    if (threadIdx.x == 2)
+        __hip_atomic_store(&blk->look_tick, 0u, __ATOMIC_RELAXED, __HIP_MEMORY_SCOPE_AGENT);
+}
+
+void ek_launch_view_look(const float *dist0, int64_t n0, const float *dist1, int64_t n1,
+                         EkCtl *ctl, double rho, double rel, double abs_, hipStream_t s)
+{
+    if (n0 <= 0)
+        return;
+    const unsigned nb0 = (unsigned)((n0 + EK_VIEW_LOOK_SEL - 1) / EK_VIEW_LOOK_SEL);
+    const unsigned nb1 =
+        n1 > 0 ? (unsigned)((n1 + EK_VIEW_LOOK_SEL - 1) / EK_VIEW_LOOK_SEL) : 0u;
+    hipLaunchKernelGGL(ek_view_look_kernel, dim3(nb0 + nb1), dim3(EK_BLOCK), 0, s, dist0, n0,
+                       nb0, dist1, n1, (EkCtlBlock *)ctl, rho, rel, abs_);
 }
 
 __global__ void __launch_bounds__(EK_BLOCK)
diff --git a/enspara_amd/device.py b/enspara_amd/device.py
--- a/enspara_amd/device.py
+++ b/enspara_amd/device.py
@@ -485,6 +485,15 @@
         return {"views": int(s[0]), "streamed": int(s[1]), "left_out": int(s[2]),
                 "guard_exits": int(s[3])}
 
+    def run_loop_stats(self):
+        s = np.zeros(13, dtype=np.int64)
+        _lib.check(self.lib.ek_run_loop_stats(self._h, _lib.i64p(s)))
+        return {"host_waits": int(s[0]),
+                "batches": {T: int(s[1 + k]) for k, T in enumerate((1, 4, 8, 16, 32))},
+                "longest_batch": int(s[6]), "probes_up": (int(s[7]), int(s[8])),
+                "probes_down": (int(s[9]), int(s[10])), "bootstraps": int(s[11]),
+                "looks": int(s[12])}
+
     def last_run_form(self):
         s = np.zeros(6, dtype=np.int64)
         _lib.check(self.lib.ek_last_run_form(self._h, _lib.i64p(s)))
diff --git a/include/enspara_hip.h b/include/enspara_hip.h
--- a/include/enspara_hip.h
+++ b/include/enspara_hip.h
@@ -89,6 +89,7 @@
 int ek_run_stats(ek_ctx *ctx, int64_t *passes, int64_t *centers);
 int ek_ti_stats(ek_ctx *ctx, int64_t *tiles, int64_t *skipped);
 int ek_view_stats(ek_ctx *ctx, int64_t *stats);
+int ek_run_loop_stats(ek_ctx *ctx, int64_t *out);
 int ek_last_run_form(ek_ctx *ctx, int64_t *out);
 int ek_view_layout_check(ek_ctx *ctx, float theta, int64_t *out);
 
```
